# carlobaldassi/GaussDCA.jl

Hardware: AMD Instinct MI355X
Metric: end-to-end gDCA sec + achieved Cholesky TFLOP/s, N=500 M=50k q=21 (higher is better)
Workload: dtype f64

## Files before the change

### gaussdca.jl_amd/csrc/gdca_api.hip

```cpp
#include <algorithm>
#include <ctype.h>
#include <math.h>
#include <stdio.h>
#include <stdlib.h>
#include <string.h>
#include <strings.h>

#include "gdca_hamming_form.h"
#include "gdca_internal.h"
#include "gdca_launch.h"

struct gdca_buf {
    void *p;
    size_t cap;
};

class stage_pool {
    friend class host_stage;
    static const int MAX_ARRAYS = 10;
    gdca_buf buf[MAX_ARRAYS];

public:
    void release()
    {
// ... 530 lines not shown
{
    return (int32_t)sizeof(gdca_params);
}

int32_t gdca_device_count(void)
{
    int n = 0;
    if (hipGetDeviceCount(&n) != hipSuccess) return 0;
    return n;
}

gdca_status gdca_ctx_create_on_stream(int32_t device_id, void *hip_stream, gdca_ctx **out)
{
    if (!out) return GDCA_EINVAL;
    *out = nullptr;
    int ndev = 0;
    if (hipGetDeviceCount(&ndev) != hipSuccess || ndev <= 0) return GDCA_EHIP;
    if (device_id < 0 || device_id >= ndev) return GDCA_EINVAL;
    gdca_ctx *ctx = (gdca_ctx *)calloc(1, sizeof(gdca_ctx));
    if (!ctx) return GDCA_ENOMEM;
    ctx->device = device_id;
    ctx->timing = true;
    gdca_tuning_from_env(&ctx->tune);
    if (hipSetDevice(device_id) != hipSuccess) {
        free(ctx);
        return GDCA_EHIP;
    }
    ctx->stream = (hipStream_t)hip_stream;
    ctx->own_stream = false;
    {
        hipDeviceProp_t prop0;
        ctx->ncu = hipGetDeviceProperties(&prop0, device_id) == hipSuccess ? prop0.multiProcessorCount : 256;
    }
    if (hipEventCreateWithFlags(&ctx->ev_batch, hipEventDisableTiming) != hipSuccess ||
        hipEventCreateWithFlags(&ctx->ev_upload, hipEventDisableTiming) != hipSuccess) {
        gdca_ctx_destroy(ctx);
        return GDCA_EHIP;
    }
    if (hipHostMalloc((void **)&ctx->sc_host, sizeof(gdca_dev_scalars), hipHostMallocDefault) != hipSuccess) {
        ctx->sc_host = nullptr;
        gdca_ctx_destroy(ctx);
        return GDCA_ENOMEM;
    }
    if (hipHostGetDevicePointer((void **)&ctx->sc_host_dev, ctx->sc_host, 0) != hipSuccess) ctx->sc_host_dev = nullptr;
    *out = ctx;
    return GDCA_OK;
}

static gdca_status warm_stream(gdca_ctx *ctx, hipStream_t s)
{
    CHK(ensure(ctx, ctx->sc, sizeof(gdca_dev_scalars)));
    gdca_fill_async(s, ctx->sc.p, 0, sizeof(gdca_dev_scalars));
    if (hipStreamSynchronize(s) != hipSuccess) {
        (void)hipGetLastError();
        return fail(ctx, GDCA_EHIP, "the context's stream could not be started");
    }
    return GDCA_OK;
}

gdca_status gdca_ctx_create(int32_t device_id, gdca_ctx **out)
{
    gdca_status st = gdca_ctx_create_on_stream(device_id, nullptr, out);
    if (st != GDCA_OK) return st;
    gdca_ctx *ctx = *out;
    int prio_least = 0, prio_greatest = 0;
    (void)hipDeviceGetStreamPriorityRange(&prio_least, &prio_greatest);
    if (hipStreamCreateWithPriority(&ctx->stream, hipStreamNonBlocking, prio_greatest) != hipSuccess) {
        gdca_ctx_destroy(ctx);
        *out = nullptr;
        return GDCA_EHIP;
    }
    ctx->own_stream = true;
    st = warm_stream(ctx, ctx->stream);
    if (st != GDCA_OK) {
        gdca_ctx_destroy(ctx);
        *out = nullptr;
    }
    return st;
}

gdca_status gdca_ctx_create_peer(gdca_ctx *leader, gdca_ctx **out)
{
    if (!leader || !out) return GDCA_EINVAL;
    gdca_ctx *ctx = leader;
    HIPCHK(hipSetDevice(leader->device));
    if (!leader->gate) {
        gdca_gate *g = (gdca_gate *)calloc(1, sizeof(gdca_gate));
        if (!g) return GDCA_ENOMEM;
        for (int i = 0; i < 4; ++i) HIPCHK(hipEventCreateWithFlags(&g->ev[i], hipEventDisableTiming));
        g->refs = 1;
        int prio_least = 0, prio_greatest = 0;
        (void)hipDeviceGetStreamPriorityRange(&prio_least, &prio_greatest);
        if (hipStreamCreateWithPriority(&g->batch_stream, hipStreamNonBlocking, prio_greatest) != hipSuccess) g->batch_stream = nullptr;
        leader->gate = g;
    }
    const bool new_gate = leader->gate->refs == 1;
    gdca_status st = gdca_ctx_create(leader->device, out);
    if (st != GDCA_OK) return st;
    (*out)->gate = leader->gate;
    leader->gate->refs += 1;
    if (new_gate && leader->gate->batch_stream) {
        st = warm_stream(*out, leader->gate->batch_stream);
        if (st != GDCA_OK) {
            gdca_ctx_destroy(*out);
            *out = nullptr;
        }
    }
    return st;
}

gdca_status gdca_ctx_destroy(gdca_ctx *ctx)
{
    if (!ctx) return GDCA_EINVAL;
    (void)hipSetDevice(ctx->device);
    if (ctx->own_stream || ctx->stream) (void)hipStreamSynchronize(ctx->stream);
    gdca_buf *bufs[] = {&ctx->Zt, &ctx->Zp, &ctx->hist, &ctx->Zb, &ctx->hcnt, &ctx->nk, &ctx->W, &ctx->Wfix, &ctx->Pifix,
                        &ctx->Pipc, &ctx->A, &ctx->G, &ctx->H, &ctx->P, &ctx->Sg, &ctx->Dblk, &ctx->Ld,
                        &ctx->Tws, &ctx->colsum, &ctx->sc, &ctx->normws, &ctx->C2, &ctx->B0, &ctx->Rt, &ctx->Wd, &ctx->rankws, &ctx->hcand, &ctx->himg,
                        &ctx->Pij, &ctx->sc_front, &ctx->keep, &ctx->Xg, &ctx->Epart, &ctx->gpart, &ctx->gvec,
                        &ctx->PXa, &ctx->PXb, &ctx->PXpad, &ctx->PEab, &ctx->PT, &ctx->PBtab, &ctx->PBitems, &ctx->PBE,
                        &ctx->LOa, &ctx->LOb, &ctx->PBN,
                        &ctx->IPAws, &ctx->IPAcnt, &ctx->IPAZ, &ctx->IPAsel, &ctx->IPAm, &ctx->IPAg, &ctx->IPAprev, &ctx->IPAsp, &ctx->DMd, &ctx->SMst, &ctx->BMws, &ctx->BMred};
    for (gdca_buf *b : bufs)
        if (b->p) (void)hipFree(b->p);
    ctx->staging.release();
    if (ctx->gate && --ctx->gate->refs == 0) {
        for (int i = 0; i < 4; ++i) (void)hipEventDestroy(ctx->gate->ev[i]);
        if (ctx->gate->batch_stream) {
            (void)hipStreamSynchronize(ctx->gate->batch_stream);
            (void)hipStreamDestroy(ctx->gate->batch_stream);
        }
        free(ctx->gate);
    }
    for (hipEvent_t e : ctx->ev)
        if (e) (void)hipEventDestroy(e);
    if (ctx->item0_host) (void)hipHostFree(ctx->item0_host);
    if (ctx->ev_batch) (void)hipEventDestroy(ctx->ev_batch);
    if (ctx->ev_upload) (void)hipEventDestroy(ctx->ev_upload);
    if (ctx->sc_host) (void)hipHostFree(ctx->sc_host);
    if (ctx->own_stream) (void)hipStreamDestroy(ctx->stream);
    free(ctx);
    return GDCA_OK;
}

gdca_status gdca_ctx_synchronize(gdca_ctx *ctx)
{
    if (!ctx) return GDCA_EINVAL;
    HIPCHK(hipSetDevice(ctx->device));
    HIPCHK(hipStreamSynchronize(ctx->stream));
    return GDCA_OK;
}

const char *gdca_last_error(gdca_ctx *ctx)
{
    return ctx ? ctx->err : "null context";
}

gdca_status gdca_ctx_set_timing(gdca_ctx *ctx, int32_t enabled)
{
    if (!ctx) return GDCA_EINVAL;
    ctx->timing = enabled != 0;
    return GDCA_OK;
}

gdca_status gdca_ctx_set_option(gdca_ctx *ctx, const char *key, const char *value)
{
    if (!ctx) return GDCA_EINVAL;
    if (!key || !value) return fail(ctx, GDCA_EINVAL, "null option key or value");
    if (!gdca_tuning_set(&ctx->tune, key, value)) return fail(ctx, GDCA_EINVAL, "unknown option or unusable value: %s=%s", key, value);
    return GDCA_OK;
}

}

static gdca_status open_timeline(gdca_ctx *ctx, bool timed, bool stamped)
{
    gdca_pending &r = ctx->pend;
    r.timed = timed;
    r.stamped = stamped;
    r.ev_marks = r.stamp_marks = 0;
    for (int t = 0; timed && t < T_COUNT; ++t)
        if (!ctx->ev[t]) HIPCHK(hipEventCreate(&ctx->ev[t]));
    return GDCA_OK;
}

static void note_mark(gdca_pending &r, gdca_boundary t, bool stamp)
{
    (stamp ? r.stamp_marks : r.ev_marks) |= 1u << t;
    (stamp ? r.ev_marks : r.stamp_marks) &= ~(1u << t);
}

static gdca_status mark(gdca_ctx *ctx, gdca_boundary t, bool own_launch = false)
{
    gdca_pending &r = ctx->pend;
    if (!r.timed) return GDCA_OK;
    const bool stamp = r.stamped && !own_launch;
    if (stamp)
        gdca_launch_stamp(ctx->stream, (gdca_dev_scalars *)ctx->sc.p, t, T_NONE);
    else
        HIPCHK(hipEventRecord(ctx->ev[t], ctx->stream));
    note_mark(r, t, stamp);
    return GDCA_OK;
}

static gdca_status mark_members(hipStream_t s, gdca_ctx *const *mem, int K, gdca_boundary a, gdca_boundary b, bool stamps)
{
    gdca_ctx *ctx = mem[0];
    if (stamps) {
        gdca_recorder *&act = gdca_recorder::active();
        gdca_recorder *outer = act;
        if (outer) (void)outer->flush();
        gdca_recorder rec;
        rec.begin(s, K);
        for (int k = 0; k < K; ++k) {
            rec.member(k);
            gdca_launch_stamp(s, (gdca_dev_scalars *)mem[k]->sc.p, a, b);
        }
        (void)rec.end();
        act = outer;
    } else
        for (int k = 0; k < K; ++k) {
            HIPCHK(hipEventRecord(mem[k]->ev[a], s));
            HIPCHK(hipEventRecord(mem[k]->ev[b], s));
        }
    for (int k = 0; k < K; ++k) {
        note_mark(mem[k]->pend, a, stamps);
        note_mark(mem[k]->pend, b, stamps);
    }
    return GDCA_OK;
}

static void sweep_events(gdca_ctx *ctx, hipEvent_t *begin, hipEvent_t *end)
{
    const bool timed = ctx->pend.timed;
    *begin = timed ? ctx->ev[T_SWEEP_BEGIN] : nullptr;
    *end = timed ? ctx->ev[T_SWEEP_END] : nullptr;
    note_mark(ctx->pend, T_SWEEP_BEGIN, false);
    note_mark(ctx->pend, T_SWEEP_END, false);
}

static double elapsed(const gdca_ctx *ctx, gdca_boundary a, gdca_boundary b, bool *failed)
{
    const gdca_pending &r = ctx->pend;
    const unsigned both = 1u << a | 1u << b;
    if (!r.timed) return 0.0;
    if ((r.stamp_marks & both) == both) return (double)(long long)(ctx->sc_host->stamp[b] - ctx->sc_host->stamp[a]) * 1e-5;
    if ((r.ev_marks & both) != both) return 0.0;
    float ms = 0.f;
    if (hipEventElapsedTime(&ms, ctx->ev[a], ctx->ev[b]) != hipSuccess) *failed = true;
    return ms;
}

static hipError_t gate_wait(const gdca_gate *g, hipStream_t s)
{
    return g->armed ? hipStreamWaitEvent(s, g->ev[g->last], 0) : hipSuccess;
}

static hipError_t gate_pass(gdca_gate *g, hipStream_t s)
{
    const hipError_t e = hipEventRecord(g->ev[g->next], s);
    if (e != hipSuccess) return e;
    g->last = g->next;
    g->next = (g->next + 1) & 3;
    g->armed = 1;
    return hipSuccess;
}

static gdca_status member_error(gdca_ctx *lead, gdca_ctx *m, int k, gdca_status st)
{
    if (k > 0 && m != lead && m->err[0]) {
        char msg[sizeof(lead->err)];
        snprintf(msg, sizeof(msg), "member %d: %.400s", k, m->err);
        memcpy(lead->err, msg, sizeof(msg));
    }
    return st;
}

static gdca_status upload_done(gdca_ctx *ctx)
{
    HIPCHK(hipEventRecord(ctx->ev_upload, ctx->stream));
    HIPCHK(hipEventSynchronize(ctx->ev_upload));
    return GDCA_OK;
}

static double inverse_flops_model(double n)
{
    return (n * n * n / 3.0 + n * n / 2.0 + n / 6.0) + (2.0 * n * n * n / 3.0 + n * n / 2.0 + 5.0 * n / 6.0);
}

static int round_up(int x, int m)
{
    return (x + m - 1) / m * m;
}

static gdca_status weights_stage(gdca_ctx *ctx, const int8_t *Zd, int N, int M, int q, double theta_in, int fixed_thresh,
                                 bool want_theta_only)
{
    hipStream_t s = ctx->stream;
    gdca_dev_scalars *sc = (gdca_dev_scalars *)ctx->sc.p;
    CHK(ensure(ctx, ctx->hist, gdca_column_hist_bytes(N, M)));
    if (fixed_thresh >= 0) {
        gdca_launch_set_thresh(s, sc, fixed_thresh);
    } else {
        if (theta_in < 0.0) gdca_launch_column_hist(s, Zd, (uint32_t *)ctx->hist.p, N, M);
        gdca_launch_theta_finalize(s, (const uint32_t *)ctx->hist.p, N, M, theta_in, sc);
    }
    CHK(check_launch(ctx, "theta"));
    CHK(mark(ctx, T_THETA));
    if (want_theta_only) return GDCA_OK;

    const int Mt = (M + GDCA_HTILE - 1) / GDCA_HTILE;
    CHK(ensure(ctx, ctx->Zb, gdca_bitplane_bytes(N, M)));
    CHK(ensure(ctx, ctx->hcnt, (size_t)Mt * GDCA_HTILE * sizeof(int32_t)));
    if (!ctx->tune.force_fallback && ctx->tune.hamming_mode != 0) CHK(ensure(ctx, ctx->hcand, gdca_hamming_cand_cap(M) * 8));
    const bool fp4 = !ctx->tune.force_fallback && (ctx->tune.hamming_mode == 2 || (ctx->tune.hamming_mode < 0 && gdca_hamming_consensus_gate(N, M)));
    if (fp4) CHK(ensure(ctx, ctx->himg, gdca_fp4_image_bytes(N, M)));
    CHK(ensure(ctx, ctx->nk, (size_t)M * sizeof(int32_t)));
    CHK(ensure(ctx, ctx->W, (size_t)M * sizeof(double)));
    CHK(ensure(ctx, ctx->Wfix, (size_t)M * sizeof(unsigned long long)));
    gdca_fill_async(s, ctx->hcnt.p, 0, (size_t)Mt * GDCA_HTILE * sizeof(int32_t));
    gdca_launch_bitplane_pack(s, Zd, (uint32_t *)ctx->Zb.p, N, M, q, sc);
    if (ctx->tune.force_fallback) {
        gdca_launch_hamming_fallback(s, Zd, (int32_t *)ctx->hcnt.p, N, M, sc);
    } else {
        if (fp4) {
            if (!(fixed_thresh < 0 && theta_in < 0.0)) gdca_launch_column_hist(s, Zd, (uint32_t *)ctx->hist.p, N, M);
            gdca_launch_hamming_fp4_image(s, Zd, (const uint32_t *)ctx->hist.p, ctx->himg.p, N, M);
        }
        gdca_launch_hamming(s, (const uint32_t *)ctx->Zb.p, Zd, (int32_t *)ctx->hcnt.p, N, M, sc, ctx->tune.hamming_mode, ctx->hcand.p, fp4 ? ctx->himg.p : nullptr, ctx->tune.ham_cut);
    }
    gdca_launch_weights(s, (const int32_t *)ctx->hcnt.p, M, gdca_fix_shift(M), (int32_t *)ctx->nk.p,
                        (double *)ctx->W.p, (unsigned long long *)ctx->Wfix.p);
    gdca_launch_meff(s, (const double *)ctx->W.p, M, sc);
    return check_launch(ctx, "weights");
}

static gdca_status tally_stage(gdca_ctx *ctx, const int8_t *Zd, int N, int M, int q, const double *Meff_dev, double pc,
                               int mode, double *Pi_true_out, double *out, size_t ld, bool want_norm1 = false)
{
    hipStream_t s = ctx->stream;
    const int sdim = q - 1, n = N * sdim;
    const int shift = gdca_fix_shift(M);
    const int TJ = gdca_tally_tj(q, ctx->tune.tally_tj);
    const bool skip = gdca_tally_skip(q, TJ, ctx->tune.tally_skip, M);
    const size_t keep_list = (size_t)N * M * sizeof(uint32_t);
    if (skip) CHK(ensure(ctx, ctx->keep, keep_list + (size_t)N * sizeof(int) + N));
    CHK(ensure(ctx, ctx->Zt, (size_t)N * M + 3));
    CHK(ensure(ctx, ctx->Zp, (size_t)round_up(N, 64) * M + 64));
    CHK(ensure(ctx, ctx->Pifix, (size_t)N * 32 * sizeof(unsigned long long)));
    CHK(ensure(ctx, ctx->Pipc, (size_t)n * sizeof(double)));
    uint32_t *keep = skip ? (uint32_t *)ctx->keep.p : nullptr;
    int *keep_n = skip ? (int *)((char *)ctx->keep.p + keep_list) : nullptr;
    uint8_t *sigma = skip ? (uint8_t *)(keep_n + N) : nullptr;
    gdca_launch_relayout(s, Zd, (int8_t *)ctx->Zt.p, (int8_t *)ctx->Zp.p, N, M, TJ);
    gdca_launch_pi_keep(s, (const int8_t *)ctx->Zt.p, (const unsigned long long *)ctx->Wfix.p, (unsigned long long *)ctx->Pifix.p, keep, keep_n,
                        sigma, N, M, q, (gdca_dev_scalars *)ctx->sc.p);
    gdca_launch_pi_finalize(s, (const unsigned long long *)ctx->Pifix.p, N, q, shift, Meff_dev, pc, Pi_true_out,
                            (double *)ctx->Pipc.p, want_norm1 ? &((gdca_dev_scalars *)ctx->sc.p)->pi_max : nullptr);
    if (want_norm1) CHK(mark(ctx, T_TALLY_BEGIN));
    gdca_launch_pair_tally(s, (const int8_t *)ctx->Zp.p, (const int8_t *)ctx->Zt.p,
                           (const unsigned long long *)ctx->Wfix.p, N, M, q, shift, Meff_dev, pc,
                           (const double *)ctx->Pipc.p, mode, out, ld, TJ, keep, keep_n, sigma,
                           (const unsigned long long *)ctx->Pifix.p);
    if (want_norm1) CHK(mark(ctx, T_TALLY_END));
    if (want_norm1 && !gdca_norm1_settled(N, q, pc, ctx->tune.refine, ctx->tune.refine_cond))
        gdca_launch_cov_norm1(s, out, ld, N, q, pc, ctx->tune.refine_cond, (gdca_dev_scalars *)ctx->sc.p, ctx->tune.refine == 1);
    return check_launch(ctx, "tally");
}

static gdca_status inverse_job(gdca_ctx *ctx, int n, int n_pad, gdca_inverse_job *job)
{
    const size_t pbytes = (size_t)n_pad * GDCA_TILE * sizeof(double);
    const int nblk = n_pad / GDCA_TILE;
    const size_t sg = (size_t)4 * GDCA_TILE * 4 * GDCA_TILE * sizeof(double);
    const size_t fbytes = gdca_inverse_flag_bytes(n_pad);
    CHK(ensure(ctx, ctx->G, (size_t)8 * pbytes));
    CHK(ensure(ctx, ctx->H, (size_t)8 * pbytes));
    CHK(ensure(ctx, ctx->P, (size_t)GDCA_TILE * GDCA_TILE * sizeof(double)));
    const size_t piv_off = (4 * sg + fbytes + (size_t)3 * (nblk + 2) * sizeof(int) + 15) & ~(size_t)15;
    CHK(ensure(ctx, ctx->Sg, piv_off + (size_t)n_pad * sizeof(double)));
    if (ctx->item0_cap < 3 * (nblk + 2)) {
        if (ctx->item0_host) HIPCHK(hipHostFree(ctx->item0_host));
        ctx->item0_host = nullptr;
        ctx->item0_cap = 0;
        HIPCHK(hipHostMalloc((void **)&ctx->item0_host, (size_t)3 * (nblk + 2) * sizeof(int), hipHostMallocDefault));
        ctx->item0_cap = 3 * (nblk + 2);
    }
    gdca_inverse_ws &ws = job->ws;
    for (int w = 0; w < 8; ++w) {
        ws.G[w] = (double *)((char *)ctx->G.p + (size_t)w * pbytes);
        ws.H[w] = (double *)((char *)ctx->H.p + (size_t)w * pbytes);
    }
    ws.P = (double *)ctx->P.p;
    ws.Sg[0] = (double *)ctx->Sg.p;
    ws.Sg[1] = (double *)((char *)ctx->Sg.p + sg);
    ws.Pg[0] = (double *)((char *)ctx->Sg.p + 2 * sg);
    ws.Pg[1] = (double *)((char *)ctx->Sg.p + 3 * sg);
    ws.flags = (unsigned *)((char *)ctx->Sg.p + 4 * sg);
    ws.flags_bytes = fbytes;
    ws.item0_dev = (int *)((char *)ctx->Sg.p + 4 * sg + fbytes);
    ws.item0_host = ctx->item0_host;
    ws.piv = ctx->piv = (double *)((char *)ctx->Sg.p + piv_off);
    ctx->ld.count = 0;
    ctx->ld.chol = false;
    {
        void *dp = nullptr;
        ws.item0_host_dev = hipHostGetDevicePointer(&dp, ctx->item0_host, 0) == hipSuccess ? (const int *)dp : nullptr;
    }
    ws.update_cus = ctx->ncu;
    job->A = (double *)ctx->A.p;
    job->n_pad = n_pad;
    job->n_real = n;
    job->sc = (gdca_dev_scalars *)ctx->sc.p;
    job->tune = &ctx->tune;
    job->doomed = (ctx->tune.sweep_debug & 32) != 0 && ctx->pend.at.attempt == 0;
    return GDCA_OK;
}

static gdca_status poison_inverse_ws(gdca_ctx *ctx, hipStream_t s)
{
    HIPCHK(hipMemsetAsync(ctx->G.p, 0xFF, ctx->G.cap, s));
    HIPCHK(hipMemsetAsync(ctx->H.p, 0xFF, ctx->H.cap, s));
    HIPCHK(hipMemsetAsync(ctx->P.p, 0xFF, ctx->P.cap, s));
    HIPCHK(hipMemsetAsync(ctx->Sg.p, 0xFF, (size_t)4 * 4 * GDCA_TILE * 4 * GDCA_TILE * sizeof(double), s));
    return GDCA_OK;
}

static gdca_status inverse_stage(gdca_ctx *ctx, int n, int n_pad, double *upd_flops)
{
    gdca_inverse_job job;
    CHK(inverse_job(ctx, n, n_pad, &job));
    hipEvent_t sweep_begin, sweep_end;
    sweep_events(ctx, &sweep_begin, &sweep_end);
    if (ctx->tune.sweep_debug & 16) CHK(poison_inverse_ws(ctx, ctx->stream));
    if (ctx->tune.sweep_debug & 8) {
        double fl = 0.0;
        gdca_launch_spd_inverse_merged(ctx->stream, &job, 1, sweep_begin, sweep_end, &fl);
        if (upd_flops) *upd_flops = fl;
        return check_launch(ctx, "spd_inverse_merged");
    }
    gdca_launch_spd_inverse(ctx->stream, job, sweep_begin, sweep_end, upd_flops);
    return check_launch(ctx, "spd_inverse");
}

static gdca_status logdet_stage(gdca_ctx *ctx, int n)
{
    gdca_launch_logdet(ctx->stream, ctx->piv, n, (gdca_dev_scalars *)ctx->sc.p);
    return check_launch(ctx, "logdet");
}

static void note_logdet(gdca_ctx *ctx, int k = 0)
{
    const gdca_dev_scalars &h = *ctx->sc_host;
    ctx->ld.val[k] = h.info == 0 && !h.bad_symbol ? h.logdet : (double)NAN;
    ctx->ld.src[k] = ctx->ld.chol ? 1 : 0;
    ctx->ld.count = k + 1;
}

static gdca_status g_room(gdca_ctx *ctx, int n)
{
    const int nb = gdca_energy_gblocks(n);
    CHK(ensure(ctx, ctx->gpart, (size_t)nb * nb * 64 * sizeof(double)));
    return ensure(ctx, ctx->gvec, ((size_t)n + 1) * sizeof(double));
}

static void g_launch(gdca_ctx *ctx, const gdca_model &m)
{
    const int n = m.N * (m.q - 1);
    double *g = (double *)ctx->gvec.p;
    gdca_launch_energy_g(ctx->stream, m.A, m.ld, m.sign, n, m.Pi, (double *)ctx->gpart.p, g, g + n);
}

static gdca_status pack_and_g(gdca_ctx *ctx, const gdca_model &m, const int8_t *X_dev, int K, size_t stride = 0)
{
    CHK(ensure(ctx, ctx->Xg, (size_t)gdca_energy_blocks(m.N) * K * sizeof(uint32_t)));
    CHK(g_room(ctx, m.N * (m.q - 1)));
    gdca_launch_energy_pack(ctx->stream, X_dev, stride ? stride : (size_t)m.N, m.N, K, m.q, (uint32_t *)ctx->Xg.p, (gdca_dev_scalars *)ctx->sc.p);
    g_launch(ctx, m);
    return GDCA_OK;
}

static gdca_status energy_stage(gdca_ctx *ctx, const gdca_model &m, const int8_t *X_dev, int K, double *E_dev, size_t stride = 0)
{
    const int sdim = m.q - 1, n = m.N * sdim;
    const int Kc = gdca_energy_chunk(m.N, K, ctx->tune.energy_chunk);
    CHK(ensure(ctx, ctx->Epart, (size_t)gdca_energy_blocks(m.N) * Kc * sizeof(double)));
    CHK(pack_and_g(ctx, m, X_dev, K, stride));
    const double *g = (const double *)ctx->gvec.p;
    for (int k0 = 0; k0 < K; k0 += Kc)
        HIPCHK(gdca_launch_energy_rows(ctx->stream, m.A, m.ld, m.sign, g, g + n, (const uint32_t *)ctx->Xg.p, m.N, sdim, K, k0,
                                       std::min(Kc, K - k0), (double *)ctx->Epart.p, E_dev, ctx->ncu));
    return check_launch(ctx, "energies");
}

static gdca_status pair_pack(gdca_ctx *ctx, int N, int q, int split, const int8_t *XA, size_t strideA, int KA, const int8_t *XB, size_t strideB,
                             int KB, int what)
{
    hipStream_t s = ctx->stream;
    gdca_dev_scalars *sc = (gdca_dev_scalars *)ctx->sc.p;
    CHK(ensure(ctx, ctx->PXa, (size_t)gdca_energy_blocks(split) * KA * sizeof(uint32_t)));
    CHK(ensure(ctx, ctx->PXb, (size_t)gdca_energy_blocks(N - split) * KB * sizeof(uint32_t)));
    gdca_launch_energy_pack(s, XA, strideA, split, KA, q, (uint32_t *)ctx->PXa.p, sc);
    gdca_launch_energy_pack(s, XB, strideB, N - split, KB, q, (uint32_t *)ctx->PXb.p, sc);
    if (what == GDCA_PAIR_ENERGY) {
        CHK(ensure(ctx, ctx->PXpad, (size_t)N * ((size_t)KA + (size_t)KB)));
        gdca_launch_pair_pad(s, XA, strideA, XB, strideB, N, split, KA, KB, q, (int8_t *)ctx->PXpad.p);
    }
    return GDCA_OK;
}

static gdca_status pair_stage(gdca_ctx *ctx, const gdca_model &m, int split, const int8_t *XA, size_t strideA, int KA, const int8_t *XB,
                              size_t strideB, int KB, int what, double *E_dev, const pair_blocks *blk = nullptr, bool packed = false,
                              const gdca_logodds_terms *lo = nullptr)
{
    hipStream_t s = ctx->stream;
    const int N = m.N, q = m.q, sdim = q - 1, n = N * sdim, nB = (N - split) * sdim;
    if (!packed) CHK(pair_pack(ctx, N, q, split, XA, strideA, KA, XB, strideB, KB, what));
    const double *EAB = nullptr, *c0 = nullptr;
    if (what == GDCA_PAIR_ENERGY) {
        CHK(ensure(ctx, ctx->PEab, ((size_t)KA + (size_t)KB) * sizeof(double)));
        CHK(energy_stage(ctx, m, (const int8_t *)ctx->PXpad.p, KA + KB, (double *)ctx->PEab.p));
        EAB = (const double *)ctx->PEab.p;
        c0 = (const double *)ctx->gvec.p + n;
    }
    const int Ac = blk ? blk->Ac : gdca_pair_chunk(nB, KA, ctx->tune.pair_chunk);
    CHK(ensure(ctx, ctx->PT, (size_t)Ac * nB * sizeof(double)));
    for (int a0 = 0, c = 0; a0 < KA; a0 += Ac, ++c) {
        if (blk)
            HIPCHK(gdca_launch_pair_chunk_blocked(s, m.A, m.ld, m.sign, (const uint32_t *)ctx->PXa.p, (const uint32_t *)ctx->PXb.p, N, split, sdim,
                                                  KA, KB, a0, std::min(Ac, KA - a0), (double *)ctx->PT.p, EAB, c0, E_dev,
                                                  blk->items + 4 * blk->first[c], blk->first[c + 1] - blk->first[c], blk->eoff, blk->offA,
                                                  blk->offB, ctx->ncu, lo));
        else
            HIPCHK(gdca_launch_pair_chunk(s, m.A, m.ld, m.sign, (const uint32_t *)ctx->PXa.p, (const uint32_t *)ctx->PXb.p, N, split, sdim, KA, KB,
                                          a0, std::min(Ac, KA - a0), (double *)ctx->PT.p, EAB, c0, E_dev, ctx->ncu, lo));
    }
    return check_launch(ctx, blk ? "blocked pair energies" : "pair energies");
}

static gdca_status assign_stage(gdca_ctx *ctx, const double *E_dev, const pair_blocks &blk, int32_t *match_dev, double *gap_dev)
{
    HIPCHK(gdca_launch_assign_blocks(ctx->stream, E_dev, blk.eoff, blk.offA, blk.offB, blk.S, blk.kmax, match_dev, gap_dev));
    return check_launch(ctx, "assignment");
}

static gdca_status mutation_stage(gdca_ctx *ctx, const gdca_model &m, const int8_t *X_dev, int K, int what, double *D_dev)
{
    CHK(pack_and_g(ctx, m, X_dev, K));
    HIPCHK(gdca_launch_mutation_scan(ctx->stream, m.A, m.ld, m.sign, (const double *)ctx->gvec.p, (const uint32_t *)ctx->Xg.p, m.N, m.q - 1, K,
                                     what, D_dev, ctx->ncu));
    return check_launch(ctx, "mutation scan");
}

static gdca_status double_stage(gdca_ctx *ctx, const gdca_model &m, const int8_t *X_dev, int K, double *Emin_dev, int32_t *code_dev,
                                double *epi_dev, const int32_t *muts_dev, int L, double *out_dev)
{
    CHK(ensure(ctx, ctx->DMd, (size_t)m.q * (size_t)m.N * (size_t)K * sizeof(double)));
    CHK(mutation_stage(ctx, m, X_dev, K, GDCA_MUT_DELTA, (double *)ctx->DMd.p));
    if (muts_dev) {
        gdca_launch_double_mutants(ctx->stream, m.A, m.ld, m.sign, (const uint32_t *)ctx->Xg.p, (const double *)ctx->DMd.p, muts_dev, L, m.N,
                                   m.q - 1, K, out_dev, (gdca_dev_scalars *)ctx->sc.p);
        return check_launch(ctx, "double mutants");
    }
    HIPCHK(gdca_launch_double_mutant_scan(ctx->stream, m.A, m.ld, m.sign, (const uint32_t *)ctx->Xg.p, (const double *)ctx->DMd.p, m.N, m.q - 1,
                                          K, Emin_dev, code_dev, epi_dev, ctx->tune.epi_generic != 0));
    return check_launch(ctx, "double-mutant scan");
}

static bool walk_placement(const gdca_ctx *ctx, int N, int q, bool *in_lds)
{
    const bool fits = gdca_walk_table_fits(N, q);
    *in_lds = ctx->tune.walk_table == 2 ? false : fits;
    return fits || ctx->tune.walk_table != 1;
}

static gdca_status walk_stage(gdca_ctx *ctx, const gdca_model &m, const int8_t *X_dev, int K, const walk_request &w)
{
    bool in_lds = false;
    if (!walk_placement(ctx, m.N, m.q, &in_lds)) return fail(ctx, GDCA_EINVAL, "WALK_TABLE = lds: the table does not fit into LDS");
    double *V = w.V;
    if (!V) {
        CHK(ensure(ctx, ctx->DMd, (size_t)m.q * (size_t)m.N * (size_t)K * sizeof(double)));
        V = (double *)ctx->DMd.p;
    }
    CHK(mutation_stage(ctx, m, X_dev, K, GDCA_MUT_POTENTIAL, V));
    HIPCHK(gdca_launch_greedy_walk(ctx->stream, m.A, m.ld, m.sign, (const uint32_t *)ctx->Xg.p, m.N, m.q - 1, K, w.mask, w.flags, w.min_gain,
                                   w.max_steps, V, in_lds, w.V != nullptr, w.Xout, w.steps, w.dE_sum, w.path, w.dE_path));
    return check_launch(ctx, "greedy walk");
}

static gdca_status sample_stage(gdca_ctx *ctx, const gdca_model &m, const int8_t *X_dev, int K, const sample_request &r)
{
    bool in_lds = false;
    if (!walk_placement(ctx, m.N, m.q, &in_lds)) return fail(ctx, GDCA_EINVAL, "WALK_TABLE = lds: the table does not fit into LDS");
    double *V = r.V;
    if (!V) {
        CHK(ensure(ctx, ctx->DMd, (size_t)m.q * (size_t)m.N * (size_t)K * sizeof(double)));
        V = (double *)ctx->DMd.p;
    }
    CHK(ensure(ctx, ctx->SMst, gdca_sample_state_bytes(m.N, K)));
    CHK(mutation_stage(ctx, m, X_dev, K, GDCA_MUT_POTENTIAL, V));
    const int n_steps = r.plan.burn + r.plan.n_samples * r.plan.stride;
    const int chunk = ctx->tune.sample_chunk > 0 ? ctx->tune.sample_chunk : GDCA_SAMPLE_CHUNK_RULE;
    for (int t0 = 0; t0 < n_steps;) {
        const int t1 = n_steps - t0 > chunk ? t0 + chunk : n_steps;
        HIPCHK(gdca_launch_sample(ctx->stream, m.A, m.ld, m.sign, (const uint32_t *)ctx->Xg.p, m.N, m.q - 1, K, r.plan, t0, t1, V, in_lds,
                                  ctx->SMst.p));
        t0 = t1;
    }
    return check_launch(ctx, "Metropolis chains");
}

static gdca_status score_stage(gdca_ctx *ctx, int N, int sdim, int n_pad, const score_target &t)
{
    hipStream_t s = ctx->stream;
    const gdca_model m{(const double *)ctx->A.p, (size_t)n_pad, -1.0, (const double *)ctx->Pipc.p + (size_t)ctx->pend.site0 * sdim, N, sdim + 1};
    if (t.logodds) return GDCA_OK;
    switch (t.kind) {
    case score_target::ENERGY:
    case score_target::LOGLIK: return energy_stage(ctx, m, t.X, t.K, t.out, t.strideX);
    case score_target::PAIR: return pair_stage(ctx, m, t.split, t.XA, t.strideA, t.KA, t.XB, t.strideB, t.KB, t.what, t.out);
    case score_target::PARTNER:
        CHK(pair_stage(ctx, m, t.split, t.XA, t.strideA, t.KA, t.XB, t.strideB, t.KB, t.what, t.out, &t.blocks, t.packed));
        return assign_stage(ctx, t.out, t.blocks, t.match, t.gap);
    case score_target::MUTATION: return mutation_stage(ctx, m, t.X, t.K, t.what, t.out);
    case score_target::DOUBLE_SCAN: return double_stage(ctx, m, t.X, t.K, t.out, t.dcode, t.depi, nullptr, 0, nullptr);
    case score_target::DOUBLE_LIST: return double_stage(ctx, m, t.X, t.K, nullptr, nullptr, nullptr, t.muts, t.L, t.out);
    case score_target::WALK: return walk_stage(ctx, m, t.X, t.K, t.walk);
    case score_target::SAMPLE: return sample_stage(ctx, m, t.X, t.K, t.sample);
    case score_target::CONTACT: break;
    }
    double *S_dev = t.out;
    if (t.score == GDCA_SCORE_DI) {
        CHK(ensure(ctx, ctx->Tws, gdca_di_ws_bytes(N, sdim)));
        gdca_launch_di(s, (const double *)ctx->A.p, (size_t)n_pad, (const double *)ctx->Ld.p, N, sdim, S_dev,
                       (double *)ctx->Tws.p, (gdca_dev_scalars *)ctx->sc.p);
// ... 2942 lines not shown
```

### gaussdca.jl_amd/csrc/gdca_internal.h

```cpp
#pragma once

#include <hip/hip_runtime.h>
#include <stdint.h>

#include <vector>

#include "gdca.h"
#include "gdca_inverse_outcome.h"

#define GDCA_TILE 128
#define GDCA_HTILE 128
#define GDCA_MAXQ 31

enum gdca_boundary {
    T_NONE = -1,
    T_BEGIN, T_THETA, T_WEIGHTS,
    T_TALLY_BEGIN, T_TALLY_END,
    T_COV,
    T_INV_BEGIN, T_SWEEP_BEGIN, T_SWEEP_END, T_INV_END,
    T_SCORE_BEGIN, T_FN_BEGIN, T_FN_END, T_END,
    T_COUNT
};

struct gdca_dev_scalars {
    double theta;
    double Meff;
    unsigned long long pair_sum;
    int thresh;
    int info;
    int bad_symbol;
    int di_noconv;
    int ham_mode;
    int ham_cand;
    unsigned long long ham_ncand;
    unsigned long long sweep_cycles, sweep_ticks;
    double inv_norm1;
    double ns_resid;
    double mat_norm1;
    double pi_max;
    unsigned long long stamp[T_COUNT];
    int ham_cand2;
    int ham_cut;
    unsigned ham_alive[64];
    double logdet;
};

struct gdca_tuning {
    int group;
    int ramp;
    int ragged;
    int rem_tail;
    int panel_halves;
    int slab;
    int ring;
    int mcus;
    int mcu_solo;
    int sweep_debug;
    long sweep_timeout_ms;
    int sweep_retries;
    int tally_tj;
    int tally_skip;
    int hamming_mode;
    int ham_cut;
    int force_fallback;
    int merge;
    int merge_blocks;
    int merge_mcus;
    int merge_group;
    int merge_tiles;
    int phased_fronts;
    int phased_grids;
    int phased_streams;
    int refine;
    double refine_cond;
    int cholesky;
    int energy_chunk;
    int pair_chunk;
    int epi_generic;
    int walk_table;
    int sample_chunk;
    char sweep_trace[256];
};
void gdca_tuning_from_env(gdca_tuning *t);
bool gdca_tuning_set(gdca_tuning *t, const char *key, const char *value);

void gdca_launch_relayout(hipStream_t s, const int8_t *Z, int8_t *Zt, int8_t *Zc, int N, int M, int TJ);
size_t gdca_column_hist_bytes(int N, int M);
void gdca_launch_column_hist(hipStream_t s, const int8_t *Z, uint32_t *cnt, int N, int M);
void gdca_launch_theta_finalize(hipStream_t s, const uint32_t *cnt, int N, int M, double theta_in,
                                gdca_dev_scalars *sc);
void gdca_launch_set_thresh(hipStream_t s, gdca_dev_scalars *sc, int thresh);

size_t gdca_bitplane_bytes(int N, int M);
void gdca_launch_bitplane_pack(hipStream_t s, const int8_t *Z, uint32_t *Zb, int N, int M, int q,
                               gdca_dev_scalars *sc);
size_t gdca_hamming_cand_cap(int M);
size_t gdca_fp4_image_bytes(int N, int M);
void gdca_launch_hamming_fp4_image(hipStream_t s, const int8_t *Z, const uint32_t *hist, void *img, int N, int M);
void gdca_launch_hamming_fp4_probe(hipStream_t s, const void *img, int N, int M, int nprobe, gdca_dev_scalars *sc);
void gdca_launch_hamming_fp4(hipStream_t s, const void *img, int N, int M, gdca_dev_scalars *sc, void *cand_list, unsigned cap);
void gdca_launch_hamming(hipStream_t s, const uint32_t *Zb, const int8_t *Z, int32_t *cnt, int N, int M, gdca_dev_scalars *sc, int force,
                         void *cand_list, void *fp4_img, int cut);
void gdca_launch_hamming_fallback(hipStream_t s, const int8_t *Z, int32_t *cnt, int N, int M, const gdca_dev_scalars *sc);
void gdca_launch_weights(hipStream_t s, const int32_t *cnt, int M, int fix_shift, int32_t *n_out, double *W,
                         unsigned long long *Wfix);
void gdca_launch_meff(hipStream_t s, const double *W, int M, gdca_dev_scalars *sc);
void gdca_launch_fix_weights(hipStream_t s, const double *W, int M, int fix_shift, unsigned long long *Wfix,
                             gdca_dev_scalars *sc);
int gdca_fix_shift(int M);

void gdca_launch_pi_keep(hipStream_t s, const int8_t *Zt, const unsigned long long *Wfix, unsigned long long *Pifix, uint32_t *keep,
                         int *keep_n, uint8_t *sigma, int N, int M, int q, gdca_dev_scalars *sc);
void gdca_launch_pi_finalize(hipStream_t s, const unsigned long long *Pifix, int N, int q, int fix_shift,
                             const double *Meff_dev, double pc, double *Pi_true, double *Pi_pc, double *pi_max = nullptr);
void gdca_launch_cov_norm1(hipStream_t s, const double *C, size_t ld, int N, int q, double pc, double cond_limit, gdca_dev_scalars *sc,
                           int always);
int gdca_tally_tj(int q, int tj_wanted);
bool gdca_tally_skip(int q, int TJ, int skip_wanted, int M);
void gdca_launch_pair_tally(hipStream_t s, const int8_t *Zc, const int8_t *Zt, const unsigned long long *Wfix,
                            int N, int M, int q, int fix_shift, const double *Meff_dev, double pc,
                            const double *Pi_pc, int mode, double *out, size_t ld, int TJ, const uint32_t *keep = nullptr,
                            const int *keep_n = nullptr, const uint8_t *sigma = nullptr, const unsigned long long *Pifix = nullptr);
void gdca_launch_cov_from_pij(hipStream_t s, const double *Pij, const double *Pi_pc, int N, int q, double pc, double *out, size_t ld,
                              size_t ldp = 0);

void gdca_launch_add_pseudocount(hipStream_t s, const double *Pi_true, const double *Pij_true, int N, int q,
                                 double pc, double *Pi, double *Pij);
void gdca_launch_covariance(hipStream_t s, const double *Pi, const double *Pij, int n, double *C);
void gdca_launch_pad_identity(hipStream_t s, double *A, int n, int n_pad);
void gdca_launch_copy_in(hipStream_t s, const double *src, int n, double *dst, int n_pad);
void gdca_launch_copy_in_neg(hipStream_t s, const double *src, int n, double *dst, int n_pad);
void gdca_launch_copy_out_neg_sym(hipStream_t s, const double *A, int n_pad, double *dst, int n);
void gdca_launch_publish_scalars(hipStream_t s, const gdca_dev_scalars *sc, gdca_dev_scalars *host_mapped);
void gdca_launch_save_diag_blocks(hipStream_t s, const double *C, size_t ld, int N, int sdim, double *D);

struct gdca_inverse_ws {
    double *G[8];
    double *H[8];
    double *P;
    double *piv;
    double *Sg[2];
    double *Pg[2];
    unsigned *flags;
    size_t flags_bytes;
    int *item0_host;
    const int *item0_host_dev;
    int *item0_dev;
    int update_cus;
};
struct gdca_inverse_job {
    double *A;
    int n_pad, n_real;
    gdca_inverse_ws ws;
    gdca_dev_scalars *sc;
    const gdca_tuning *tune;
    bool doomed;
};
size_t gdca_inverse_flag_bytes(int n_pad);
void gdca_launch_spd_inverse(hipStream_t s, const gdca_inverse_job &job, hipEvent_t sweep_begin, hipEvent_t sweep_end, double *upd_flops);
int gdca_inverse_max_merge(void);
void gdca_launch_spd_inverse_merged(hipStream_t s, const gdca_inverse_job *jobs, int K, hipEvent_t sweep_begin, hipEvent_t sweep_end,
                                    double *upd_flops);
size_t gdca_ranking_ws_bytes(long long len);
void gdca_launch_ranking(hipStream_t s, const double *S_dev, int N, int sep, long long len, void *ws, int32_t **ii, int32_t **jj, double **sc);
__device__ __forceinline__ uint64_t gdca_rank_key(double x)
{
    const uint64_t u = (uint64_t)__double_as_longlong(x);
    uint64_t asc = (u >> 63) ? ~u : (u | 0x8000000000000000ull);
    if (x != x) asc = ~0ull;
    return ~asc;
}
size_t gdca_sort_hist_words(size_t n);
void gdca_launch_sort_pairs(hipStream_t s, uint64_t *const key[2], uint32_t *const val[2], uint32_t *hist, size_t n);
void gdca_launch_probe_mfma_f64(hipStream_t s, double *out, int iters, int blocks);
void gdca_launch_cholesky_inverse(hipStream_t s, double *C2, double *U, double *Tm, double *Wd, double *Aout, int n_pad, int n_real,
                                  gdca_dev_scalars *sc, double *piv);
void gdca_launch_inverse_norm1(hipStream_t s, const double *A, int n_pad, int n, double *colsum_ws, double *out);
void gdca_launch_matrix_norm1(hipStream_t s, const double *C, size_t ld, int n, double *colsum_ws, double *out);
void gdca_launch_newton_schulz(hipStream_t s, double *A, const double *C2, double *B0, double *Rt, int n_pad, double *resid);

void gdca_launch_logdet(hipStream_t s, const double *piv, int n_real, gdca_dev_scalars *sc);
void gdca_launch_loglik(hipStream_t s, double *L, int K, double c);

void gdca_launch_fn(hipStream_t s, const double *A, size_t ld, int N, int sdim, double *S, int ncu = 0);
void gdca_launch_diag_chol(hipStream_t s, const double *D, int N, int sdim, double *Ld);
size_t gdca_di_ws_bytes(int N, int sdim);
void gdca_launch_di(hipStream_t s, const double *A, size_t ld, const double *Ld, int N, int sdim, double *S,
                    double *Tws, gdca_dev_scalars *sc);
void gdca_launch_apc(hipStream_t s, double *S, int N, double *rowsum_ws);

struct gdca_model {
    const double *A;
    size_t ld;
    double sign;
    const double *Pi;
    int N, q;
};

int gdca_energy_blocks(int Ns);
int gdca_energy_gblocks(int n);
int gdca_energy_chunk(int N, int K, int wanted);
void gdca_launch_energy_pack(hipStream_t s, const int8_t *X, size_t stride, int Ns, int K, int q, uint32_t *Xg, gdca_dev_scalars *sc);
void gdca_launch_energy_g(hipStream_t s, const double *A, size_t ld, double sign, int n, const double *Pi, double *part, double *g,
                          double *c0);
hipError_t gdca_launch_energy_rows(hipStream_t s, const double *A, size_t ld, double sign, const double *g, const double *c0,
                                   const uint32_t *Xg, int N, int sdim, int K, int k0, int Kc, double *part, double *E, int ncu);

int gdca_pair_chunk(int nB, int KA, int wanted);
void gdca_launch_pair_pad(hipStream_t s, const int8_t *XA, size_t strideA, const int8_t *XB, size_t strideB, int N, int split, int KA, int KB,
                          int q, int8_t *Xp);
struct gdca_logodds_terms {
    const double *EmA, *EmB;
    double I;
};
hipError_t gdca_launch_pair_chunk(hipStream_t s, const double *A, size_t ld, double sign, const uint32_t *XAg, const uint32_t *XBg, int N,
                                  int split, int sdim, int KA, int KB, int a0, int Ac, double *T, const double *EAB, const double *c0, double *E,
                                  int ncu, const gdca_logodds_terms *lo = nullptr);
void gdca_pair_block_items(const int32_t *offA, const int32_t *offB, int S, int Ac, std::vector<int32_t> &items, std::vector<long long> &first);
hipError_t gdca_launch_pair_chunk_blocked(hipStream_t s, const double *A, size_t ld, double sign, const uint32_t *XAg, const uint32_t *XBg, int N,
                                          int split, int sdim, int KA, int KB, int a0, int Ac, double *T, const double *EAB, const double *c0,
                                          double *E, const int32_t *items, long long nitems, const long long *eoff, const int32_t *offA,
                                          const int32_t *offB, int ncu, const gdca_logodds_terms *lo = nullptr);
void gdca_launch_negate(hipStream_t s, const double *src, double *dst, size_t len);

hipError_t gdca_launch_assign_blocks(hipStream_t s, const double *E, const long long *eoff, const int32_t *offA, const int32_t *offB, int S,
                                     int kmax, int32_t *match, double *gap);

struct gdca_ipa_counts {
    double cost;
    int n_changed;
    int ncand;
    int n_sel;
    int pad_;
};
size_t gdca_ipa_select_ws_bytes(int KA);
void gdca_launch_ipa_select(hipStream_t s, const int32_t *match, const double *gap, int KA, int n_take, void *ws, int32_t *sel, gdca_ipa_counts *out);
void gdca_launch_ipa_concat(hipStream_t s, const int8_t *XA, int KA, const int8_t *XB, int KB, int N, int split, const int32_t *selA,
                            const int32_t *selB, const int32_t *viaB, int n_sel, int8_t *Z, size_t col0, gdca_dev_scalars *sc);
void gdca_launch_ipa_round(hipStream_t s, const double *E, const long long *eoff, const int32_t *offA, const int32_t *offB, const int32_t *spA,
                           const int32_t *match, const int32_t *prev, int KA, gdca_ipa_counts *out);
void gdca_launch_ipa_publish(hipStream_t s, const int32_t *match, const double *gap, int KA, int32_t *prev, int32_t *match_out, double *gap_out,
                             int32_t *match_row, double *gap_row);

hipError_t gdca_launch_mutation_scan(hipStream_t s, const double *A, size_t ld, double sign, const double *g, const uint32_t *Xg, int N, int sdim,
                               int K, int what, double *D, int ncu);

#define GDCA_EPI_MAX_GROUPS (1LL << 24)
hipError_t gdca_launch_double_mutant_scan(hipStream_t s, const double *A, size_t ld, double sign, const uint32_t *Xg, const double *D, int N,
                                          int sdim, int K, double *Emin, int32_t *code, double *epi, bool generic);
void gdca_launch_double_mutants(hipStream_t s, const double *A, size_t ld, double sign, const uint32_t *Xg, const double *D,
                                const int32_t *muts, long long L, int N, int sdim, int K, double *out, gdca_dev_scalars *sc);

#define GDCA_WALK_LDS_LIMIT (160 * 1024)
size_t gdca_walk_lds_bytes(int N, int q, bool table_in_lds);
bool gdca_walk_table_fits(int N, int q);
hipError_t gdca_launch_greedy_walk(hipStream_t s, const double *A, size_t ld, double sign, const uint32_t *Xg, int N, int sdim, int K,
                                   const int8_t *mask, int flags, double min_gain, int max_steps, double *V, bool table_in_lds, bool write_table,
                                   int8_t *Xout, int32_t *steps, double *dE_sum, int32_t *path, double *dE_path);

#define GDCA_SAMPLE_CHUNK_RULE 65536
struct gdca_sample_plan {
    const int8_t *mask;
    int flags;
    double beta;
    unsigned long long seed, stream0;
    int burn, stride, n_samples;
    int8_t *Xs;
    double *dE_s;
    int32_t *accepted;
    double *thr;
    int32_t *moves;
};
size_t gdca_sample_lds_bytes(int N, int q, bool table_in_lds);
size_t gdca_sample_state_bytes(int N, int K);
hipError_t gdca_launch_sample(hipStream_t s, const double *A, size_t ld, double sign, const uint32_t *Xg, int N, int sdim, int K,
                              const gdca_sample_plan &plan, int t0, int t1, double *V, bool table_in_lds, void *state);

void gdca_launch_bm_from_gaussian(hipStream_t s, const double *mJ, const double *g, int N, int sdim, double *W);
void gdca_launch_bm_update(hipStream_t s, double *W, const double *Pij_d, const double *Pij_m, int N, int sdim, double eta, double lambda);
size_t gdca_bm_readout_bytes(int n);
void gdca_launch_bm_readout(hipStream_t s, const double *Pi_d, const double *Pij_d, const double *Pi_m, const double *Pij_m, int N, int sdim,
                            double *part, double *out, bool zero3);
void gdca_launch_bm_accept(hipStream_t s, const int32_t *accepted, int K, long long n_steps, double *out);
void gdca_launch_bm_last_sample(hipStream_t s, const int8_t *Xs, int N, int K, int n_samples, int8_t *X);
void gdca_launch_bm_fill(hipStream_t s, double *v, size_t count, double value);
```

### gaussdca.jl_amd/csrc/k_hamming.hip

```cpp
#include <algorithm>
#include <cstdlib>

#include "gdca_hamming_cut.h"
#include "gdca_hamming_form.h"
#include "gdca_internal.h"
#include "gdca_launch.h"

#define NPLANES 5
#define WCHUNK 8

size_t gdca_bitplane_bytes(int N, int M)
{
    const size_t Mt = (M + GDCA_HTILE - 1) / GDCA_HTILE, NW = (N + 31) / 32;
    return Mt * NPLANES * NW * GDCA_HTILE * sizeof(uint32_t);
}

struct k_bitplane_pack_args {
    const int8_t *Z;
    uint32_t *Zb;
    int N;
    int M;
    int NW;
    int q;
    gdca_dev_scalars *sc;
};
static inline k_bitplane_pack_args k_bitplane_pack_mk(const int8_t *Z, uint32_t *Zb, int N, int M, int NW, int q, gdca_dev_scalars *sc)
{
    return k_bitplane_pack_args{Z, Zb, N, M, NW, q, sc};
}
template <int CAP>
__global__ __launch_bounds__(128) void k_bitplane_pack(const BatchArgs<k_bitplane_pack_args, CAP> B_)
{
    GDCA_MEMBER(B_);
    const int8_t *__restrict__ Z = a_.Z;
    uint32_t *__restrict__ Zb = a_.Zb;
    int N = a_.N;
    int M = a_.M;
    int NW = a_.NW;
    int q = a_.q;
    gdca_dev_scalars *sc = a_.sc;
    uint32_t bad = 0;
    const uint32_t over = (0x7fu - (uint32_t)q) * 0x01010101u;
    const int tile = blockIdx.x, w = blockIdx.y, kl = threadIdx.x;
    const int k = tile * GDCA_HTILE + kl;
    uint32_t pl[NPLANES];
#pragma unroll
    for (int p = 0; p < NPLANES; ++p) pl[p] = 0;
    if (k < M) {
        const int8_t *src = Z + (size_t)k * N + (size_t)w * 32;
        const int nb = min(32, N - w * 32);
        if (nb == 32 && (N & 3) == 0) {
            const uint32_t *s4 = reinterpret_cast<const uint32_t *>(src);
            uint32_t d[8];
#pragma unroll
            for (int j = 0; j < 8; ++j) d[j] = s4[j];
#pragma unroll
            for (int j = 0; j < 8; ++j) {
                bad |= (d[j] - 0x01010101u) & ~d[j] & 0x80808080u;
                bad |= (((d[j] & 0x7f7f7f7fu) + over) | d[j]) & 0x80808080u;
            }
#pragma unroll
            for (int j = 0; j < 8; ++j)
#pragma unroll
                for (int p = 0; p < NPLANES; ++p) {
                    const uint32_t t = (d[j] >> p) & 0x01010101u;
                    pl[p] |= (((t * 0x01020408u) >> 24) & 0xFu) << (4 * j);
                }
        } else {
            for (int b = 0; b < nb; ++b) {
                const uint32_t raw = (uint32_t)(uint8_t)src[b];
                bad |= (raw - 1u) >= (uint32_t)q;
                const uint32_t z = raw & 31u;
#pragma unroll
                for (int p = 0; p < NPLANES; ++p) pl[p] |= ((z >> p) & 1u) << b;
            }
        }
    }
#pragma unroll
    for (int p = 0; p < NPLANES; ++p)
        Zb[(((size_t)tile * NPLANES + p) * NW + w) * GDCA_HTILE + kl] = pl[p];
    if (bad) atomicOr(&sc->bad_symbol, GDCA_BAD_ALIGNMENT);
}

void gdca_launch_bitplane_pack(hipStream_t s, const int8_t *Z, uint32_t *Zb, int N, int M, int q, gdca_dev_scalars *sc)
{
    const int Mt = (M + GDCA_HTILE - 1) / GDCA_HTILE, NW = (N + 31) / 32;
    (gdca_launch<k_bitplane_pack_args, k_bitplane_pack<1>, k_bitplane_pack<GDCA_MAXB>>(dim3(Mt, NW), dim3(128), 0, s, k_bitplane_pack_mk(Z, Zb, N, M, NW, q, sc)));
}

__device__ __forceinline__ void tri_decode(int t, int Mt, int &I, int &J)
{
    const double b = 2.0 * Mt + 1.0;
    int i = (int)((b - sqrt(b * b - 8.0 * (double)t)) * 0.5);
    if (i < 0) i = 0;
    if (i > Mt - 1) i = Mt - 1;
    auto start = [Mt](int r) { return (long long)r * Mt - (long long)r * (r - 1) / 2; };
    while (i > 0 && start(i) > t) --i;
    while (i < Mt - 1 && start(i + 1) <= t) ++i;
    I = i;
    J = i + (int)(t - start(i));
}

#define HAM_BOUND_PLANES 3
#define HAM_CAND_CAP 1024

__shared__ int hm_any[3];
__shared__ unsigned hm_tile_n, hm_tile_base;
__shared__ uint32_t hm_list[4][HAM_LIST_WAVE];
__shared__ int hm_wave_n[4];
__shared__ unsigned hm_alive[HAM_ALIVE_SLOTS];
#define HAM_ENT_DIST 0x3ffffu
#define HAM_NO_PAIR 0x40000000u
static_assert(sizeof(((gdca_dev_scalars *)nullptr)->ham_alive) == HAM_ALIVE_SLOTS * sizeof(unsigned), "one slot per word the probe counts");
__device__ __forceinline__ bool wg_any(bool pred, int &k)
{
    const int s = k % 3, n = (k + 1) % 3;
    ++k;
    if (threadIdx.x == 0) hm_any[n] = 0;
    if (__any(pred) && (threadIdx.x & 63) == 0) atomicOr(&hm_any[s], 1);
    __syncthreads();
    return hm_any[s] != 0;
}


size_t gdca_hamming_cand_cap(int M)
{
    const long long Mt = (M + GDCA_HTILE - 1) / GDCA_HTILE;
    return (size_t)std::min<long long>(Mt * (Mt + 1) / 2 * HAM_CAND_PER_TILE + 4096, 1ll << 30);
}

struct k_hamming_refine_args {
    const int8_t *Z;
    const int2 *list;
    unsigned cap;
    int N;
    int32_t *cnt;
    const gdca_dev_scalars *sc;
};
static inline k_hamming_refine_args k_hamming_refine_mk(const int8_t *Z, const int2 *list, unsigned cap, int N, int32_t *cnt, const gdca_dev_scalars *sc)
{
    return k_hamming_refine_args{Z, list, cap, N, cnt, sc};
}
template <int CAP>
__global__ __launch_bounds__(256) void k_hamming_refine(const BatchArgs<k_hamming_refine_args, CAP> B_)
{
    GDCA_MEMBER(B_);
    const int8_t *__restrict__ Z = a_.Z;
    const int2 *__restrict__ list = a_.list;
    unsigned cap = a_.cap;
    int N = a_.N;
    int32_t *__restrict__ cnt = a_.cnt;
    const gdca_dev_scalars *__restrict__ sc = a_.sc;
    if (sc->ham_mode == 0) return;
    if (sc->ham_ncand > (unsigned long long)cap) return;
    const unsigned total = (unsigned)sc->ham_ncand;
    const int thresh = sc->thresh;
    const int tid = threadIdx.x, sub = tid & 15, grp = (tid & 63) >> 4;
    const unsigned wave = blockIdx.x * 4u + (unsigned)(tid >> 6), nwave = gridDim.x * 4u;
    for (unsigned eb = wave * 4u; eb < total; eb += nwave * 4u) {
        const unsigned e = eb + (unsigned)grp;
        uint32_t d = 0;
        int k = 0, l = 0;
        if (e < total) {
            const int2 pr = list[e];
            k = pr.x;
            l = pr.y;
            const int8_t *zk = Z + (size_t)k * N, *zl = Z + (size_t)l * N;
            if ((N & 3) == 0 && (reinterpret_cast<uintptr_t>(Z) & 3) == 0) {
                const uint32_t *a = reinterpret_cast<const uint32_t *>(zk), *b = reinterpret_cast<const uint32_t *>(zl);
                const int nw = N >> 2;
                for (int w0 = 0; w0 < nw; w0 += 256) {
                    uint32_t xa[16], xb[16];
#pragma unroll
                    for (int u = 0; u < 16; ++u) {
                        const int w = w0 + 16 * u + sub;
                        xa[u] = w < nw ? a[w] : 0u;
                        xb[u] = w < nw ? b[w] : 0u;
                    }
#pragma unroll
                    for (int u = 0; u < 16; ++u) {
                        uint32_t x = xa[u] ^ xb[u];
                        x |= x >> 4;
                        x |= x >> 2;
                        x |= x >> 1;
                        d += __builtin_popcount(x & 0x01010101u);
                    }
                }
            } else {
                for (int i = sub; i < N; i += 16) d += zk[i] != zl[i];
            }
        }
        d += __shfl_xor(d, 1);
        d += __shfl_xor(d, 2);
        d += __shfl_xor(d, 4);
        d += __shfl_xor(d, 8);
        if (e < total && sub == 0 && (int)d < thresh) {
            atomicAdd(&cnt[k], 1);
            atomicAdd(&cnt[l], 1);
        }
    }
}

struct k_hamming_args {
    const uint32_t *Zb;
    int32_t *cnt;
    int NW;
    int M;
    int Mt;
    gdca_dev_scalars *sc;
    int2 *cand_list;
    unsigned cand_cap;
};
static inline k_hamming_args k_hamming_mk(const uint32_t *Zb, int32_t *cnt, int NW, int M, int Mt, gdca_dev_scalars *sc, int2 *cand_list, unsigned cand_cap)
{
    return k_hamming_args{Zb, cnt, NW, M, Mt, sc, cand_list, cand_cap};
}
template <int CAP, int NP, bool PROBE>
__global__ __launch_bounds__(256, (NP < NPLANES && !PROBE) ? 4 : 3) void k_hamming(const BatchArgs<k_hamming_args, CAP> B_)
{
    GDCA_MEMBER(B_);
    const uint32_t *__restrict__ Zb = a_.Zb;
    int32_t *__restrict__ cnt = a_.cnt;
    int NW = a_.NW;
    int M = a_.M;
    int Mt = a_.Mt;
    gdca_dev_scalars *__restrict__ sc = a_.sc;
    int2 *__restrict__ cand_list = a_.cand_list;
    unsigned cand_cap = a_.cand_cap;
    const int thresh = sc->thresh;
    if (thresh <= 0) return;
    if constexpr (!PROBE) {
        const bool mine = NP == NPLANES ? (sc->ham_mode == 0 || sc->ham_ncand > cand_cap) : sc->ham_mode == 1;
        if (!mine) return;
    }

    __shared__ __attribute__((aligned(16))) uint32_t As[NP][WCHUNK][GDCA_HTILE];
    __shared__ __attribute__((aligned(16))) uint32_t Bs[NP][WCHUNK][GDCA_HTILE];
    __shared__ int rc[GDCA_HTILE], cc[GDCA_HTILE];

    int I, J;
    tri_decode(PROBE ? (int)(((long long)blockIdx.x * ((long long)Mt * (Mt + 1) / 2)) / gridDim.x) : (int)blockIdx.x, Mt, I, J);
    const int tid = threadIdx.x, tx = tid & 15, ty = tid >> 4;
    if (tid < GDCA_HTILE) {
        rc[tid] = 0;
        cc[tid] = 0;
    }
    if (tid == 0) {
        hm_any[0] = 0;
        hm_any[1] = 0;
        hm_tile_n = 0u;
    }
    int any_calls = 0;

    uint32_t acc[8][8];
#pragma unroll
    for (int r = 0; r < 8; ++r)
#pragma unroll
        for (int c = 0; c < 8; ++c) acc[r][c] = 0;
    if constexpr (NP < NPLANES) {
        if (I == J || (J + 1) * GDCA_HTILE > M) {
#pragma unroll
            for (int r = 0; r < 8; ++r)
#pragma unroll
                for (int c = 0; c < 8; ++c) {
                    const int lc = (c < 4) ? (tx * 4 + c) : (64 + tx * 4 + (c - 4));
                    const int gr = I * GDCA_HTILE + ty * 8 + r, gc = J * GDCA_HTILE + lc;
                    acc[r][c] = (gr < M && gc < M && (I == J ? (PROBE ? gr != gc : gr < gc) : true)) ? 0u : HAM_NO_PAIR;
                }
        }
    }
    bool all_beyond = false;

    const uint32_t *Ag = Zb + (size_t)I * NPLANES * NW * GDCA_HTILE;
    const uint32_t *Bg = Zb + (size_t)J * NPLANES * NW * GDCA_HTILE;

    constexpr bool CUTTING = NP < NPLANES && !PROBE;
    int cut = NW;
    if constexpr (CUTTING) {
        const int c = sc->ham_cut;
        if (c > 0 && c < NW && NW < HAM_CUT_MAX_NW) cut = c;
    }
    bool sparse = false;
    if constexpr (PROBE)
        if (tid < HAM_ALIVE_SLOTS) hm_alive[tid] = 0u;

    auto stage = [&](int w0) {
#pragma unroll
        for (int p = 0; p < NP; ++p) {
            const int wl = tid >> 5;
            uint4 va = make_uint4(0, 0, 0, 0), vb = make_uint4(0, 0, 0, 0);
            if (w0 + wl < NW) {
                const size_t off = ((size_t)p * NW + w0 + wl) * GDCA_HTILE + (size_t)(tid & 31) * 4;
                va = *reinterpret_cast<const uint4 *>(Ag + off);
                vb = *reinterpret_cast<const uint4 *>(Bg + off);
            }
            *reinterpret_cast<uint4 *>(&As[p][wl][(tid & 31) * 4]) = va;
            *reinterpret_cast<uint4 *>(&Bs[p][wl][(tid & 31) * 4]) = vb;
        }
    };

    int w0 = 0;
    for (; w0 < NW; w0 += WCHUNK) {
        __syncthreads();
        stage(w0);
        __syncthreads();
        const int wn = min(WCHUNK, NW - w0);
        int w = 0;
        bool again;
        do {
        again = false;
        for (const int wend = CUTTING ? min(wn, cut - w0) : wn; w < wend; ++w) {
            uint32_t a[NP][8], b[NP][8];
#pragma unroll
            for (int p = 0; p < NP; ++p) {
                const uint4 a0 = *reinterpret_cast<const uint4 *>(&As[p][w][ty * 8]);
                const uint4 a1 = *reinterpret_cast<const uint4 *>(&As[p][w][ty * 8 + 4]);
                const uint4 b0 = *reinterpret_cast<const uint4 *>(&Bs[p][w][tx * 4]);
                const uint4 b1 = *reinterpret_cast<const uint4 *>(&Bs[p][w][64 + tx * 4]);
                a[p][0] = a0.x; a[p][1] = a0.y; a[p][2] = a0.z; a[p][3] = a0.w;
                a[p][4] = a1.x; a[p][5] = a1.y; a[p][6] = a1.z; a[p][7] = a1.w;
                b[p][0] = b0.x; b[p][1] = b0.y; b[p][2] = b0.z; b[p][3] = b0.w;
                b[p][4] = b1.x; b[p][5] = b1.y; b[p][6] = b1.z; b[p][7] = b1.w;
            }
#pragma unroll
            for (int r = 0; r < 8; ++r)
#pragma unroll
                for (int c = 0; c < 8; ++c) {
                    uint32_t x = a[0][r] ^ b[0][c];
#pragma unroll
                    for (int p = 1; p < NP; ++p)
                        x = __builtin_amdgcn_bitop3_b32(a[p][r], b[p][c], x, 0xBE);
                    acc[r][c] += __builtin_popcount(x);
                }
            if constexpr (PROBE) {
                if (w0 + w < HAM_ALIVE_SLOTS) {
                    int alive = 0;
#pragma unroll
                    for (int r = 0; r < 8; ++r)
#pragma unroll
                        for (int c = 0; c < 8; ++c) alive += __builtin_popcountll(__ballot((int)acc[r][c] < thresh));
                    if ((tid & 63) == 0 && alive) atomicAdd(&hm_alive[w0 + w], (unsigned)alive);
                }
            }
        }
        if constexpr (CUTTING) {
            if (w0 + w == cut && cut < NW) {
                const uint32_t rc0 = ((uint32_t)(ty * 8) << 25) | ((uint32_t)(tx * 4) << 18);
                uint32_t *const mylist = hm_list[tid >> 6];
                int wcount = 0;
#pragma unroll
                for (int r = 0; r < 8; ++r)
#pragma unroll
                    for (int c = 0; c < 8; ++c) {
                        const bool lv = (int)acc[r][c] < thresh;
                        const unsigned long long m = __ballot(lv);
                        if (m != 0ull) {
                            if (lv) {
                                const int pos = wcount + (int)__builtin_amdgcn_mbcnt_hi((unsigned)(m >> 32), __builtin_amdgcn_mbcnt_lo((unsigned)m, 0u));
                                const uint32_t rc = ((uint32_t)r << 25) | ((uint32_t)((c < 4) ? c : 64 + (c - 4)) << 18);
                                if (pos < HAM_LIST_WAVE) mylist[pos] = acc[r][c] + (rc0 + rc);
                            }
                            wcount += __builtin_popcountll(m);
                        }
                    }
                if ((tid & 63) == 0) hm_wave_n[tid >> 6] = wcount;
                __syncthreads();
                const int n0 = hm_wave_n[0], n1 = hm_wave_n[1], n2 = hm_wave_n[2], n3 = hm_wave_n[3];
                if (max(max(n0, n1), max(n2, n3)) > HAM_LIST_WAVE) {
                    cut = NW;
                    again = w < wn;
                } else if ((n0 | n1 | n2 | n3) == 0) {
                    all_beyond = true;
                } else {
                    sparse = true;
                }
            }
        }
        } while (again);
        if (CUTTING && (sparse || all_beyond)) break;
        if (w0 + WCHUNK < NW) {
            uint32_t mn = acc[0][0];
#pragma unroll
            for (int r = 0; r < 8; ++r)
#pragma unroll
                for (int c = 0; c < 8; ++c) mn = min(mn, acc[r][c]);
            if (!wg_any((int)mn < thresh, any_calls)) {
                all_beyond = true;
                break;
            }
        }
    }

    const bool diag = (I == J);
    if constexpr (PROBE) {
        int cand = 0;
#pragma unroll
        for (int r = 0; r < 8; ++r)
#pragma unroll
            for (int c = 0; c < 8; ++c) {
                const int lc = (c < 4) ? (tx * 4 + c) : (64 + tx * 4 + (c - 4));
                const int gr = I * GDCA_HTILE + ty * 8 + r, gc = J * GDCA_HTILE + lc;
                cand += (gr < M) && (gc < M) && (gr != gc) && ((int)acc[r][c] < thresh);
            }
        if (cand) atomicAdd(&rc[0], cand);
        __syncthreads();
        if (tid == 0 && rc[0]) atomicAdd(&sc->ham_cand, rc[0]);
        if (tid < HAM_ALIVE_SLOTS && hm_alive[tid]) atomicAdd(&sc->ham_alive[tid], hm_alive[tid]);
        return;
    }
    if (all_beyond) return;
    if constexpr (CUTTING) {
        if (sparse) {
            const int lane = tid & 63, nmine = hm_wave_n[tid >> 6];
            uint32_t *const mylist = hm_list[tid >> 6];
            for (int ws = cut; ws < NW; ws = w0 + WCHUNK) {
                if (ws >= w0 + WCHUNK) {
                    w0 += WCHUNK;
                    __syncthreads();
                    stage(w0);
                    __syncthreads();
                }
                const int wn = min(WCHUNK, NW - w0);
                bool left = false;
                for (int e = lane; e < nmine; e += 64) {
                    const uint32_t ent = mylist[e];
                    uint32_t d = ent & HAM_ENT_DIST;
                    if ((int)d < thresh) {
                        const int row = (int)(ent >> 25), col = (int)((ent >> 18) & 127u);
                        for (int w = ws - w0; w < wn; ++w) {
                            uint32_t x = As[0][w][row] ^ Bs[0][w][col];
#pragma unroll
                            for (int p = 1; p < NP; ++p) x = __builtin_amdgcn_bitop3_b32(As[p][w][row], Bs[p][w][col], x, 0xBE);
                            d += __builtin_popcount(x);
                        }
                        mylist[e] = (ent & ~HAM_ENT_DIST) | d;
                        left |= (int)d < thresh;
                    }
                }
                if (w0 + WCHUNK < NW && !wg_any(left, any_calls)) return;
            }
            unsigned mine = 0u;
            for (int e = lane; e < nmine; e += 64) mine += (int)(mylist[e] & HAM_ENT_DIST) < thresh;
            if (!wg_any(mine != 0u, any_calls)) return;
            const unsigned off = mine ? atomicAdd(&hm_tile_n, mine) : 0u;
            __syncthreads();
            if (tid == 0) {
                const unsigned long long base = atomicAdd(&sc->ham_ncand, (unsigned long long)hm_tile_n);
                hm_tile_base = base > (unsigned long long)cand_cap ? cand_cap : (unsigned)base;
            }
            __syncthreads();
            unsigned slot = hm_tile_base + off;
            for (int e = lane; e < nmine; e += 64) {
                const uint32_t ent = mylist[e];
                if ((int)(ent & HAM_ENT_DIST) < thresh) {
                    if (slot < cand_cap) cand_list[slot] = make_int2(I * GDCA_HTILE + (int)(ent >> 25), J * GDCA_HTILE + (int)((ent >> 18) & 127u));
                    ++slot;
                }
            }
            return;
        }
    }
    if constexpr (NP < NPLANES) {
        uint32_t mn = acc[0][0];
#pragma unroll
        for (int r = 0; r < 8; ++r)
#pragma unroll
            for (int c = 0; c < 8; ++c) mn = min(mn, acc[r][c]);
        unsigned long long cand = 0ull;
        if ((int)mn < thresh) {
#pragma unroll
            for (int r = 0; r < 8; ++r)
#pragma unroll
                for (int c = 0; c < 8; ++c) {
                    const int lc = (c < 4) ? (tx * 4 + c) : (64 + tx * 4 + (c - 4));
                    const int gr = I * GDCA_HTILE + ty * 8 + r, gc = J * GDCA_HTILE + lc;
                    if ((int)acc[r][c] < thresh && gr < M && gc < M && (diag ? gr < gc : true)) cand |= 1ull << (8 * r + c);
                }
        }
        if (!wg_any(cand != 0ull, any_calls)) return;
        const unsigned mine = (unsigned)__builtin_popcountll(cand);
        const unsigned off = mine ? atomicAdd(&hm_tile_n, mine) : 0u;
        __syncthreads();
        if (tid == 0) {
            const unsigned long long base = atomicAdd(&sc->ham_ncand, (unsigned long long)hm_tile_n);
            hm_tile_base = base > (unsigned long long)cand_cap ? cand_cap : (unsigned)base;
        }
        __syncthreads();
        unsigned slot = hm_tile_base + off;
        while (cand) {
            const int e = __builtin_ctzll(cand), r = e >> 3, c = e & 7;
            const int lc = (c < 4) ? (tx * 4 + c) : (64 + tx * 4 + (c - 4));
            if (slot < cand_cap) cand_list[slot] = make_int2(I * GDCA_HTILE + ty * 8 + r, J * GDCA_HTILE + lc);
            ++slot;
            cand &= cand - 1;
        }
        return;
    }

    if constexpr (NP == NPLANES) {
        int rowc[8], colc[8];
#pragma unroll
        for (int r = 0; r < 8; ++r) rowc[r] = 0;
#pragma unroll
        for (int c = 0; c < 8; ++c) colc[c] = 0;
#pragma unroll
        for (int r = 0; r < 8; ++r) {
            const int gr = I * GDCA_HTILE + ty * 8 + r;
#pragma unroll
            for (int c = 0; c < 8; ++c) {
                const int lc = (c < 4) ? (tx * 4 + c) : (64 + tx * 4 + (c - 4));
                const int gc = J * GDCA_HTILE + lc;
                const bool ok = (gr < M) && (gc < M) && (gr != gc) && ((int)acc[r][c] < thresh);
                rowc[r] += ok ? 1 : 0;
                colc[c] += ok ? 1 : 0;
            }
        }
#pragma unroll
        for (int r = 0; r < 8; ++r)
            if (rowc[r]) atomicAdd(&rc[ty * 8 + r], rowc[r]);
        if (!diag) {
#pragma unroll
            for (int c = 0; c < 8; ++c) {
                const int lc = (c < 4) ? (tx * 4 + c) : (64 + tx * 4 + (c - 4));
                if (colc[c]) atomicAdd(&cc[lc], colc[c]);
            }
        }
    }
    __syncthreads();
    if (tid < GDCA_HTILE) {
        const int v = rc[tid];
        if (v) atomicAdd(&cnt[I * GDCA_HTILE + tid], v);
    } else if (!diag) {
        const int v = cc[tid - GDCA_HTILE];
        if (v) atomicAdd(&cnt[J * GDCA_HTILE + tid - GDCA_HTILE], v);
    }
}

struct k_hamming_decide_args {
    gdca_dev_scalars *sc;
    long long sampled_pairs;
    int force;
    int consensus;
    int N, M;
    int cut;
};
static inline k_hamming_decide_args k_hamming_decide_mk(gdca_dev_scalars *sc, long long sampled_pairs, int force, int consensus, int N, int M, int cut)
{
    return k_hamming_decide_args{sc, sampled_pairs, force, consensus, N, M, cut};
}
template <int CAP>
__global__ void k_hamming_decide(const BatchArgs<k_hamming_decide_args, CAP> B_)
{
    GDCA_MEMBER(B_);
    gdca_dev_scalars *sc = a_.sc;
    long long sampled_pairs = a_.sampled_pairs;
    int force = a_.force;
    if (threadIdx.x == 0 && blockIdx.x == 0) {
        const double pairs = (double)sampled_pairs;
        const int NW = (a_.N + 31) / 32;
        const int cut = a_.cut > 0 ? a_.cut : (force < 0 ? gdca_hamming_pick_cut(sc->ham_alive, pairs, NW) : NW);
        sc->ham_cut = cut;
        sc->ham_mode = force >= 0 ? force : gdca_hamming_pick_form((double)sc->ham_cand, a_.consensus ? (double)sc->ham_cand2 : -1.0, pairs, a_.N, a_.M, cut);
        sc->ham_ncand = 0u;
    }
}

void gdca_launch_hamming(hipStream_t s, const uint32_t *Zb, const int8_t *Z, int32_t *cnt, int N, int M, gdca_dev_scalars *sc, int force,
                         void *cand_list, void *fp4_img, int cut)
{
    const int Mt = (M + GDCA_HTILE - 1) / GDCA_HTILE, NW = (N + 31) / 32;
    const long long ntile = (long long)Mt * (Mt + 1) / 2;
    int2 *list = (int2 *)cand_list;
    const unsigned cap = (unsigned)gdca_hamming_cand_cap(M);
    const int nprobe = (int)std::min<long long>(ntile, 192);
    if (force == 2 && !fp4_img) force = 1;
    if (force < 0 && NW <= 2) force = 0;
    if (force < 0 && ntile >= 64) {
        (gdca_launch<k_hamming_args, k_hamming<1, HAM_BOUND_PLANES, true>, k_hamming<GDCA_MAXB, HAM_BOUND_PLANES, true>>(dim3((unsigned)nprobe), dim3(256), 0, s, k_hamming_mk(Zb, cnt, NW, M, Mt, sc, list, cap)));
        if (fp4_img) gdca_launch_hamming_fp4_probe(s, fp4_img, N, M, nprobe, sc);
        (gdca_launch<k_hamming_decide_args, k_hamming_decide<1>, k_hamming_decide<GDCA_MAXB>>(dim3(1), dim3(1), 0, s, k_hamming_decide_mk(sc, (long long)nprobe * GDCA_HTILE * GDCA_HTILE, -1, fp4_img ? 1 : 0, N, M, cut)));
    } else {
        (gdca_launch<k_hamming_decide_args, k_hamming_decide<1>, k_hamming_decide<GDCA_MAXB>>(dim3(1), dim3(1), 0, s, k_hamming_decide_mk(sc, 1ll, force < 0 ? 0 : force, 0, N, M, cut)));
    }
    const bool decided = !(force < 0 && ntile >= 64);
    const int form = decided ? (force < 0 ? 0 : force) : -1;
    if (fp4_img && (form == 2 || form < 0)) gdca_launch_hamming_fp4(s, fp4_img, N, M, sc, list, cap);
    if (form == 1 || form < 0)
        (gdca_launch<k_hamming_args, k_hamming<1, HAM_BOUND_PLANES, false>, k_hamming<GDCA_MAXB, HAM_BOUND_PLANES, false>>(dim3((unsigned)ntile), dim3(256), 0, s, k_hamming_mk(Zb, cnt, NW, M, Mt, sc, list, cap)));
    if (form != 0)
        (gdca_launch<k_hamming_refine_args, k_hamming_refine<1>, k_hamming_refine<GDCA_MAXB>>(dim3(2048), dim3(256), 0, s, k_hamming_refine_mk(Z, (const int2 *)list, cap, N, cnt, (const gdca_dev_scalars *)sc)));
    (gdca_launch<k_hamming_args, k_hamming<1, NPLANES, false>, k_hamming<GDCA_MAXB, NPLANES, false>>(dim3((unsigned)ntile), dim3(256), 0, s, k_hamming_mk(Zb, cnt, NW, M, Mt, sc, list, cap)));
}

struct k_hamming_bytes_args {
    const int8_t *Z;
    int32_t *cnt;
    int N;
    int M;
    const gdca_dev_scalars *sc;
};
static inline k_hamming_bytes_args k_hamming_bytes_mk(const int8_t *Z, int32_t *cnt, int N, int M, const gdca_dev_scalars *sc)
{
    return k_hamming_bytes_args{Z, cnt, N, M, sc};
}
template <int CAP>
__global__ __launch_bounds__(256) void k_hamming_bytes(const BatchArgs<k_hamming_bytes_args, CAP> B_)
{
    GDCA_MEMBER(B_);
    const int8_t *__restrict__ Z = a_.Z;
    int32_t *__restrict__ cnt = a_.cnt;
    int N = a_.N;
    int M = a_.M;
    const gdca_dev_scalars *sc = a_.sc;
    extern __shared__ int8_t zk[];
    __shared__ int red[256];
    const int k = blockIdx.x, tid = threadIdx.x, thresh = sc->thresh;
    for (int i = tid; i < N; i += 256) zk[i] = Z[(size_t)k * N + i];
    __syncthreads();
    int mine = 0;
    for (int l = tid; l < M; l += 256) {
        if (l == k) continue;
        const int8_t *zl = Z + (size_t)l * N;
        int d = 0;
        for (int i = 0; i < N; ++i) d += (zl[i] != zk[i]);
        mine += (d < thresh);
    }
    red[tid] = mine;
    __syncthreads();
    for (int w = 128; w > 0; w >>= 1) {
        if (tid < w) red[tid] += red[tid + w];
        __syncthreads();
    }
    if (tid == 0) cnt[k] = red[0];
}

void gdca_launch_hamming_fallback(hipStream_t s, const int8_t *Z, int32_t *cnt, int N, int M, const gdca_dev_scalars *sc)
{
    (gdca_launch<k_hamming_bytes_args, k_hamming_bytes<1>, k_hamming_bytes<GDCA_MAXB>>(dim3((unsigned)M), dim3(256), (size_t)N, s, k_hamming_bytes_mk(Z, cnt, N, M, sc)));
}

int gdca_fix_shift(int M)
{
    int lg = 0;
    while ((1ll << lg) < (long long)M) ++lg;
    const int sh = 63 - lg;
    return sh < 58 ? sh : 58;
}

struct k_weights_args {
    const int32_t *cnt;
    int M;
    int fix_shift;
    int32_t *n_out;
    double *W;
    unsigned long long *Wfix;
};
static inline k_weights_args k_weights_mk(const int32_t *cnt, int M, int fix_shift, int32_t *n_out, double *W, unsigned long long *Wfix)
{
    return k_weights_args{cnt, M, fix_shift, n_out, W, Wfix};
}
template <int CAP>
__global__ __launch_bounds__(256) void k_weights(const BatchArgs<k_weights_args, CAP> B_)
{
    GDCA_MEMBER(B_);
    const int32_t *__restrict__ cnt = a_.cnt;
    int M = a_.M;
    int fix_shift = a_.fix_shift;
    int32_t *__restrict__ n_out = a_.n_out;
    double *__restrict__ W = a_.W;
    unsigned long long *__restrict__ Wfix = a_.Wfix;
    const int k = blockIdx.x * 256 + threadIdx.x;
    if (k >= M) return;
    const int n = 1 + cnt[k];
    if (n_out) n_out[k] = n;
    const double w = 1.0 / (double)n;
    W[k] = w;
    if (Wfix) Wfix[k] = (unsigned long long)rint(ldexp(w, fix_shift));
}

void gdca_launch_weights(hipStream_t s, const int32_t *cnt, int M, int fix_shift, int32_t *n_out, double *W,
                         unsigned long long *Wfix)
{
    (gdca_launch<k_weights_args, k_weights<1>, k_weights<GDCA_MAXB>>(dim3((M + 255) / 256), dim3(256), 0, s, k_weights_mk(cnt, M, fix_shift, n_out, W, Wfix)));
}

struct k_fix_weights_args {
    const double *W;
    int M;
    int fix_shift;
    unsigned long long *Wfix;
    gdca_dev_scalars *sc;
};
static inline k_fix_weights_args k_fix_weights_mk(const double *W, int M, int fix_shift, unsigned long long *Wfix, gdca_dev_scalars *sc)
{
    return k_fix_weights_args{W, M, fix_shift, Wfix, sc};
}
template <int CAP>
__global__ __launch_bounds__(256) void k_fix_weights(const BatchArgs<k_fix_weights_args, CAP> B_)
{
    GDCA_MEMBER(B_);
    const double *__restrict__ W = a_.W;
    int M = a_.M;
    int fix_shift = a_.fix_shift;
    unsigned long long *__restrict__ Wfix = a_.Wfix;
    gdca_dev_scalars *sc = a_.sc;
    const int k = blockIdx.x * 256 + threadIdx.x;
    if (k >= M) return;
    const double w = W[k];
    const bool ok = w >= 0.0 && w <= 1.0;
    if (!ok) atomicOr(&sc->bad_symbol, GDCA_BAD_WEIGHT);
    Wfix[k] = ok ? (unsigned long long)rint(ldexp(w, fix_shift)) : 0ull;
}

void gdca_launch_fix_weights(hipStream_t s, const double *W, int M, int fix_shift, unsigned long long *Wfix,
                             gdca_dev_scalars *sc)
{
    (gdca_launch<k_fix_weights_args, k_fix_weights<1>, k_fix_weights<GDCA_MAXB>>(dim3((M + 255) / 256), dim3(256), 0, s, k_fix_weights_mk(W, M, fix_shift, Wfix, sc)));
}

#define MEFF_FRAC 84
struct k_meff_args {
    const double *W;
    int M;
    gdca_dev_scalars *sc;
};
static inline k_meff_args k_meff_mk(const double *W, int M, gdca_dev_scalars *sc)
{
    return k_meff_args{W, M, sc};
}
template <int CAP>
__global__ __launch_bounds__(1024) void k_meff(const BatchArgs<k_meff_args, CAP> B_)
{
    GDCA_MEMBER(B_);
    const double *__restrict__ W = a_.W;
    int M = a_.M;
    gdca_dev_scalars *sc = a_.sc;
    __shared__ unsigned long long limb[3];
    const int tid = threadIdx.x;
    if (tid < 3) limb[tid] = 0ull;
    __syncthreads();
    unsigned long long l0 = 0ull, l1 = 0ull, l2 = 0ull;
    for (int k0 = tid; k0 < M; k0 += 8 * (int)blockDim.x) {
        double w[8];
#pragma unroll
        for (int u = 0; u < 8; ++u) {
            const int k = k0 + u * (int)blockDim.x;
            w[u] = k < M ? W[k] : 0.0;
        }
#pragma unroll
        for (int u = 0; u < 8; ++u) {
        const unsigned long long b = (unsigned long long)__double_as_longlong(w[u]);
        const int E = (int)((b >> 52) & 0x7ffull);
        unsigned long long m = b & 0xfffffffffffffull;
        int sh = E - 1075 + MEFF_FRAC;
        if (E != 0) m |= 1ull << 52; else sh += 1;
        if (sh < 0) {
            m = sh > -64 ? m >> (-sh) : 0ull;
            sh = 0;
        }
        if (sh > 43) sh = 43;
        const unsigned long long lo = m << sh, hi = sh ? m >> (64 - sh) : 0ull;
        l0 += lo & 0xffffffffull;
        l1 += lo >> 32;
        l2 += hi;
        }
    }
#pragma unroll
    for (int o = 32; o >= 1; o >>= 1) {
        l0 += __shfl_xor(l0, o);
        l1 += __shfl_xor(l1, o);
        l2 += __shfl_xor(l2, o);
    }
    if ((tid & 63) == 0) {
        atomicAdd(&limb[0], l0);
        atomicAdd(&limb[1], l1);
        atomicAdd(&limb[2], l2);
    }
    __syncthreads();
    if (tid == 0) {
        unsigned long long lo = limb[0], hi = limb[2];
        const unsigned long long mid = limb[1];
        const unsigned long long add = mid << 32;
        lo += add;
        hi += (mid >> 32) + (lo < add ? 1ull : 0ull);
        double r;
        if (hi == 0ull && lo < (1ull << 53)) {
            r = ldexp((double)lo, -MEFF_FRAC);
        } else {
            const int p = hi ? 127 - __builtin_clzll(hi) : 63 - __builtin_clzll(lo);
            const int shift = p - 52;
            unsigned long long kept, rem_hi, rem_lo, half_hi, half_lo;
            if (shift >= 64) {
                kept = hi >> (shift - 64);
                rem_hi = shift > 64 ? hi & ((1ull << (shift - 64)) - 1ull) : 0ull;
                rem_lo = lo;
            } else {
                kept = (lo >> shift) | (hi << (64 - shift));
                rem_hi = 0ull;
                rem_lo = lo & ((1ull << shift) - 1ull);
            }
            if (shift - 1 >= 64) {
                half_hi = 1ull << (shift - 1 - 64);
                half_lo = 0ull;
            } else {
                half_hi = 0ull;
                half_lo = 1ull << (shift - 1);
            }
            const bool above = rem_hi > half_hi || (rem_hi == half_hi && rem_lo > half_lo);
            const bool tie = rem_hi == half_hi && rem_lo == half_lo;
            if (above || (tie && (kept & 1ull))) ++kept;
            r = ldexp((double)kept, shift - MEFF_FRAC);
        }
        sc->Meff = r;
    }
}

void gdca_launch_meff(hipStream_t s, const double *W, int M, gdca_dev_scalars *sc)
{
    (gdca_launch<k_meff_args, k_meff<1>, k_meff<GDCA_MAXB>>(dim3(1), dim3(1024), 0, s, k_meff_mk(W, M, sc)));
}
```

### gaussdca.jl_amd/csrc/k_theta.hip

```cpp
#include "gdca_internal.h"
#include "gdca_launch.h"

struct k_relayout_args {
    const int8_t *Z;
    int8_t *Zt;
    int8_t *Zc;
    int N;
    int M;
    int TJ;
};
static inline k_relayout_args k_relayout_mk(const int8_t *Z, int8_t *Zt, int8_t *Zc, int N, int M, int TJ)
{
    return k_relayout_args{Z, Zt, Zc, N, M, TJ};
}
template <int CAP>
__global__ __launch_bounds__(256) void k_relayout(const BatchArgs<k_relayout_args, CAP> B_)
{
    GDCA_MEMBER(B_);
    const int8_t *__restrict__ Z = a_.Z;
    int8_t *__restrict__ Zt = a_.Zt;
    int8_t *__restrict__ Zc = a_.Zc;
    int N = a_.N;
    int M = a_.M;
    int TJ = a_.TJ;
    __shared__ uint32_t tile[64][17];
    const int k0 = blockIdx.y * 64, c0 = blockIdx.x * 64;
    const int t = threadIdx.x;
    if (((N & 3) == 0) && ((reinterpret_cast<uintptr_t>(Z) & 3) == 0)) {
        const int d = t & 15, c = c0 + 4 * d;
#pragma unroll
        for (int r = 0; r < 4; ++r) {
            const int kl = r * 16 + (t >> 4), k = k0 + kl;
            uint32_t v = 0;
            if (k < M && c < N) v = *reinterpret_cast<const uint32_t *>(Z + (size_t)k * N + c);
            tile[kl][d] = v;
        }
    } else {
        uint8_t *tb = reinterpret_cast<uint8_t *>(&tile[0][0]);
        const int tx = t & 63, ty = t >> 6;
#pragma unroll
        for (int r = 0; r < 16; ++r) {
            const int kl = r * 4 + ty, k = k0 + kl, c = c0 + tx;
            tb[kl * 68 + tx] = (k < M && c < N) ? (uint8_t)Z[(size_t)k * N + c] : (uint8_t)0;
        }
    }
    __syncthreads();
    {
        const int q16 = TJ >> 4;
        const int blk = t / (64 * q16), rem = t % (64 * q16);
        const int kl = rem / q16, h = rem % q16;
        const int k = k0 + kl, cb = c0 / TJ + blk;
        if (k < M && cb * TJ < N) {
            const int d0 = blk * (TJ >> 2) + 4 * h;
            const uint4 v = make_uint4(tile[kl][d0], tile[kl][d0 + 1], tile[kl][d0 + 2], tile[kl][d0 + 3]);
            *reinterpret_cast<uint4 *>(Zc + ((size_t)cb * M + k) * TJ + 16 * h) = v;
        }
    }
    {
        const bool wide = ((M & 3) == 0) && ((reinterpret_cast<uintptr_t>(Zt) & 3) == 0);
        const int bk = t & 15, bc = t >> 4;
        uint32_t r[4];
#pragma unroll
        for (int j = 0; j < 4; ++j) r[j] = tile[4 * bk + j][bc];
        const int k = k0 + 4 * bk;
#pragma unroll
        for (int j = 0; j < 4; ++j) {
            const int i = c0 + 4 * bc + j;
            const uint32_t o = ((r[0] >> (8 * j)) & 255u) | (((r[1] >> (8 * j)) & 255u) << 8) | (((r[2] >> (8 * j)) & 255u) << 16) |
                               (((r[3] >> (8 * j)) & 255u) << 24);
            if (i < N && k < M) {
                int8_t *dst = Zt + (size_t)i * M + k;
                if (wide) {
                    *reinterpret_cast<uint32_t *>(dst) = o;
                } else {
#pragma unroll
                    for (int e = 0; e < 4; ++e)
                        if (k + e < M) dst[e] = (int8_t)((o >> (8 * e)) & 255u);
                }
            }
        }
    }
}

void gdca_launch_relayout(hipStream_t s, const int8_t *Z, int8_t *Zt, int8_t *Zc, int N, int M, int TJ)
{
    dim3 grid((N + 63) / 64, (M + 63) / 64);
    (gdca_launch<k_relayout_args, k_relayout<1>, k_relayout<GDCA_MAXB>>(grid, dim3(256), 0, s, k_relayout_mk(Z, Zt, Zc, N, M, TJ)));
}

#define HIST_THREADS 1024
#define HIST_ROWS 8
struct k_column_hist_args {
    const int8_t *Z;
    uint32_t *out;
    int N;
    int M;
    int seq_per_block;
};
static inline k_column_hist_args k_column_hist_mk(const int8_t *Z, uint32_t *out, int N, int M, int seq_per_block)
{
    return k_column_hist_args{Z, out, N, M, seq_per_block};
}
template <int CAP>
__global__ __launch_bounds__(HIST_THREADS) void k_column_hist(const BatchArgs<k_column_hist_args, CAP> B_)
{
    GDCA_MEMBER(B_);
    const int8_t *__restrict__ Z = a_.Z;
    uint32_t *__restrict__ out = a_.out;
    int N = a_.N;
    int M = a_.M;
    int seq_per_block = a_.seq_per_block;
    constexpr int NW = HIST_THREADS / 64;
    static_assert(HIST_THREADS >= 512, "the store of the counts takes 512 threads");
    __shared__ __attribute__((aligned(16))) uint32_t h[32 * 256];
    const int t = threadIdx.x, lane = t & 63, wv = t >> 6;
    for (int e = t; e < 32 * 256; e += HIST_THREADS) h[e] = 0;
    const int c = blockIdx.x * 256 + 4 * lane;
    const int nv = N - c < 4 ? N - c : 4;
    const int kbeg = blockIdx.y * seq_per_block;
    const int kend = min(M, kbeg + seq_per_block);
    const bool wide = ((N & 3) == 0) && ((reinterpret_cast<uintptr_t>(Z) & 3) == 0);
    __syncthreads();
    if (nv > 0) {
        for (int k = kbeg + wv; k < kend; k += NW * HIST_ROWS) {
            uint32_t v[HIST_ROWS];
#pragma unroll
            for (int u = 0; u < HIST_ROWS; ++u) {
                const int ku = k + u * NW;
                v[u] = 0;
                if (ku < kend) {
                    const int8_t *p = Z + (size_t)ku * N + c;
                    if (wide) {
                        v[u] = *reinterpret_cast<const uint32_t *>(p);
                    } else {
#pragma unroll
                        for (int j = 0; j < 4; ++j)
                            if (j < nv) v[u] |= (uint32_t)(uint8_t)p[j] << (8 * j);
                    }
                }
            }
#pragma unroll
            for (int u = 0; u < HIST_ROWS; ++u) {
                if (k + u * NW < kend) {
#pragma unroll
                    for (int j = 0; j < 4; ++j)
                        if (j < nv) atomicAdd(&h[((v[u] >> (8 * j)) & 31u) * 256 + j * 64 + lane], 1u);
                }
            }
        }
    }
    __syncthreads();
    {
        const int x = t & 255, half = t >> 8;
        const int l = x & 63, j = x >> 6;
        const int col = blockIdx.x * 256 + 4 * l + j;
        if (t < 512 && col < N) {
            uint32_t *dst = out + ((size_t)blockIdx.y * N + col) * 32 + 16 * half;
#pragma unroll
            for (int g = 0; g < 4; ++g) {
                const int z = 16 * half + 4 * g;
                const uint4 o = make_uint4(h[z * 256 + j * 64 + l], h[(z + 1) * 256 + j * 64 + l], h[(z + 2) * 256 + j * 64 + l],
                                           h[(z + 3) * 256 + j * 64 + l]);
                reinterpret_cast<uint4 *>(dst)[g] = o;
            }
        }
    }
}

struct k_column_hist_sum_args {
    const uint32_t *part;
    uint32_t *cnt;
    int total;
    int chunks;
};
static inline k_column_hist_sum_args k_column_hist_sum_mk(const uint32_t *part, uint32_t *cnt, int total, int chunks)
{
    return k_column_hist_sum_args{part, cnt, total, chunks};
}
template <int CAP>
__global__ __launch_bounds__(256) void k_column_hist_sum(const BatchArgs<k_column_hist_sum_args, CAP> B_)
{
    GDCA_MEMBER(B_);
    const uint32_t *__restrict__ part = a_.part;
    uint32_t *__restrict__ cnt = a_.cnt;
    int total = a_.total;
    int chunks = a_.chunks;
    const int e = blockIdx.x * 256 + threadIdx.x;
    if (e >= total) return;
    uint32_t acc = 0;
    int c = 0;
    for (; c + 8 <= chunks; c += 8) {
        uint32_t v[8];
#pragma unroll
        for (int u = 0; u < 8; ++u) v[u] = part[(size_t)(c + u) * total + e];
#pragma unroll
        for (int u = 0; u < 8; ++u) acc += v[u];
    }
    for (; c < chunks; ++c) acc += part[(size_t)c * total + e];
    cnt[e] = acc;
}

static int column_hist_split(int N, int M, int *spb_out)
{
    const int strips = (N + 255) / 256;
    int chunks = (256 + strips - 1) / strips;
    int spb = (M + chunks - 1) / chunks;
    if (spb < 64) spb = 64;
    chunks = (M + spb - 1) / spb;
    if (spb_out) *spb_out = spb;
    return chunks;
}

size_t gdca_column_hist_bytes(int N, int M)
{
    const int chunks = column_hist_split(N, M, nullptr);
    return (size_t)N * 32 * sizeof(uint32_t) * (size_t)(chunks > 1 ? 1 + chunks : 1);
}

void gdca_launch_column_hist(hipStream_t s, const int8_t *Z, uint32_t *cnt, int N, int M)
{
    int spb;
    const int chunks = column_hist_split(N, M, &spb);
    uint32_t *out = chunks > 1 ? cnt + (size_t)N * 32 : cnt;
    (gdca_launch<k_column_hist_args, k_column_hist<1>, k_column_hist<GDCA_MAXB>>(dim3((N + 255) / 256, chunks), dim3(HIST_THREADS), 0, s, k_column_hist_mk(Z, out, N, M, spb)));
    if (chunks > 1)
        (gdca_launch<k_column_hist_sum_args, k_column_hist_sum<1>, k_column_hist_sum<GDCA_MAXB>>(dim3((N * 32 + 255) / 256, 1), dim3(256), 0, s, k_column_hist_sum_mk(out, cnt, N * 32, chunks)));
}

struct k_theta_finalize_args {
    const uint32_t *cnt;
    int N;
    int M;
    double theta_in;
    gdca_dev_scalars *sc;
};
static inline k_theta_finalize_args k_theta_finalize_mk(const uint32_t *cnt, int N, int M, double theta_in, gdca_dev_scalars *sc)
{
    return k_theta_finalize_args{cnt, N, M, theta_in, sc};
}
template <int CAP>
__global__ __launch_bounds__(256) void k_theta_finalize(const BatchArgs<k_theta_finalize_args, CAP> B_)
{
    GDCA_MEMBER(B_);
    const uint32_t *__restrict__ cnt = a_.cnt;
    int N = a_.N;
    int M = a_.M;
    double theta_in = a_.theta_in;
    gdca_dev_scalars *sc = a_.sc;
    __shared__ unsigned long long red[256];
    double theta = theta_in;
    if (theta_in < 0.0) {
        unsigned long long acc = 0;
        for (int e = threadIdx.x; e < N * 32; e += 256) {
            const unsigned long long c = cnt[e];
            acc += c * (c - 1) / 2;
        }
        red[threadIdx.x] = acc;
        __syncthreads();
        for (int w = 128; w > 0; w >>= 1) {
            if (threadIdx.x < w) red[threadIdx.x] += red[threadIdx.x + w];
            __syncthreads();
        }
        if (threadIdx.x == 0) {
            const unsigned long long tot = red[0];
            sc->pair_sum = tot;
            if (M < 2) {
                theta = 0.0;
            } else {
                const double phi = (double)tot / ((double)N * (0.5 * (double)M * (double)(M - 1)));
                const double c = 0.38 * 0.32;
                const double t = c / phi;
                theta = t < 0.5 ? t : 0.5;
            }
        }
    } else if (threadIdx.x == 0) {
        sc->pair_sum = 0;
    }
    if (threadIdx.x == 0) {
        sc->theta = theta;
        sc->thresh = (int)floor(theta * (double)N);
    }
}

void gdca_launch_theta_finalize(hipStream_t s, const uint32_t *cnt, int N, int M, double theta_in,
                                gdca_dev_scalars *sc)
{
    (gdca_launch<k_theta_finalize_args, k_theta_finalize<1>, k_theta_finalize<GDCA_MAXB>>(dim3(1), dim3(256), 0, s, k_theta_finalize_mk(cnt, N, M, theta_in, sc)));
}

struct k_set_thresh_args {
    gdca_dev_scalars *sc;
    int thresh;
};
static inline k_set_thresh_args k_set_thresh_mk(gdca_dev_scalars *sc, int thresh)
{
    return k_set_thresh_args{sc, thresh};
}
template <int CAP>
__global__ void k_set_thresh(const BatchArgs<k_set_thresh_args, CAP> B_)
{
    GDCA_MEMBER(B_);
    gdca_dev_scalars *sc = a_.sc;
    int thresh = a_.thresh;
    sc->thresh = thresh;
}

void gdca_launch_set_thresh(hipStream_t s, gdca_dev_scalars *sc, int thresh)
{
    (gdca_launch<k_set_thresh_args, k_set_thresh<1>, k_set_thresh<GDCA_MAXB>>(dim3(1), dim3(1), 0, s, k_set_thresh_mk(sc, thresh)));
}
```

Measured before the change: 52.18.

## Fuse small weight-stage kernels and make hamming kernel grid-stride persistent

Folds the theta finalize into the column histogram sum kernel using a last-block-arrives pattern, folds the hcnt zero-fill into the bitplane pack kernel, and folds the Meff reduction into the weights kernel. The hamming tile kernels become persistent, launched with a grid capped at 32 blocks per CU and looping over tiles with early exits turned into jumps to the next tile. The aim is to cut kernel-launch and tail overhead in the weights stage. The cost is extra atomics and counters in device scalars, plus a more complex control flow in the hamming kernel.

```diff
diff --git a/gaussdca.jl_amd/csrc/gdca_api.hip b/gaussdca.jl_amd/csrc/gdca_api.hip
--- a/gaussdca.jl_amd/csrc/gdca_api.hip
+++ b/gaussdca.jl_amd/csrc/gdca_api.hip
@@ -856,8 +856,8 @@
     if (fixed_thresh >= 0) {
         gdca_launch_set_thresh(s, sc, fixed_thresh);
     } else {
-        if (theta_in < 0.0) gdca_launch_column_hist(s, Zd, (uint32_t *)ctx->hist.p, N, M);
-        gdca_launch_theta_finalize(s, (const uint32_t *)ctx->hist.p, N, M, theta_in, sc);
+        const bool done = theta_in < 0.0 && gdca_launch_column_hist(s, Zd, (uint32_t *)ctx->hist.p, N, M, sc);
+        if (!done) gdca_launch_theta_finalize(s, (const uint32_t *)ctx->hist.p, N, M, theta_in, sc);
     }
     CHK(check_launch(ctx, "theta"));
     CHK(mark(ctx, T_THETA));
@@ -872,8 +872,7 @@
     CHK(ensure(ctx, ctx->nk, (size_t)M * sizeof(int32_t)));
     CHK(ensure(ctx, ctx->W, (size_t)M * sizeof(double)));
     CHK(ensure(ctx, ctx->Wfix, (size_t)M * sizeof(unsigned long long)));
-    gdca_fill_async(s, ctx->hcnt.p, 0, (size_t)Mt * GDCA_HTILE * sizeof(int32_t));
-    gdca_launch_bitplane_pack(s, Zd, (uint32_t *)ctx->Zb.p, N, M, q, sc);
+    gdca_launch_bitplane_pack(s, Zd, (uint32_t *)ctx->Zb.p, N, M, q, sc, (int32_t *)ctx->hcnt.p);
     if (ctx->tune.force_fallback) {
         gdca_launch_hamming_fallback(s, Zd, (int32_t *)ctx->hcnt.p, N, M, sc);
     } else {
@@ -881,11 +880,10 @@
             if (!(fixed_thresh < 0 && theta_in < 0.0)) gdca_launch_column_hist(s, Zd, (uint32_t *)ctx->hist.p, N, M);
             gdca_launch_hamming_fp4_image(s, Zd, (const uint32_t *)ctx->hist.p, ctx->himg.p, N, M);
         }
-        gdca_launch_hamming(s, (const uint32_t *)ctx->Zb.p, Zd, (int32_t *)ctx->hcnt.p, N, M, sc, ctx->tune.hamming_mode, ctx->hcand.p, fp4 ? ctx->himg.p : nullptr, ctx->tune.ham_cut);
+        gdca_launch_hamming(s, (const uint32_t *)ctx->Zb.p, Zd, (int32_t *)ctx->hcnt.p, N, M, sc, ctx->tune.hamming_mode, ctx->hcand.p, fp4 ? ctx->himg.p : nullptr, ctx->tune.ham_cut, ctx->ncu);
     }
     gdca_launch_weights(s, (const int32_t *)ctx->hcnt.p, M, gdca_fix_shift(M), (int32_t *)ctx->nk.p,
-                        (double *)ctx->W.p, (unsigned long long *)ctx->Wfix.p);
-    gdca_launch_meff(s, (const double *)ctx->W.p, M, sc);
+                        (double *)ctx->W.p, (unsigned long long *)ctx->Wfix.p, sc);
     return check_launch(ctx, "weights");
 }
 
diff --git a/gaussdca.jl_amd/csrc/gdca_internal.h b/gaussdca.jl_amd/csrc/gdca_internal.h
--- a/gaussdca.jl_amd/csrc/gdca_internal.h
+++ b/gaussdca.jl_amd/csrc/gdca_internal.h
@@ -43,6 +43,8 @@
     int ham_cut;
     unsigned ham_alive[64];
     double logdet;
+    unsigned long long theta_sum, meff_limb[3];
+    unsigned theta_arrived, meff_arrived;
 };
 
 struct gdca_tuning {
@@ -86,25 +88,24 @@
 
 void gdca_launch_relayout(hipStream_t s, const int8_t *Z, int8_t *Zt, int8_t *Zc, int N, int M, int TJ);
 size_t gdca_column_hist_bytes(int N, int M);
-void gdca_launch_column_hist(hipStream_t s, const int8_t *Z, uint32_t *cnt, int N, int M);
+bool gdca_launch_column_hist(hipStream_t s, const int8_t *Z, uint32_t *cnt, int N, int M, gdca_dev_scalars *sc = nullptr);
 void gdca_launch_theta_finalize(hipStream_t s, const uint32_t *cnt, int N, int M, double theta_in,
                                 gdca_dev_scalars *sc);
 void gdca_launch_set_thresh(hipStream_t s, gdca_dev_scalars *sc, int thresh);
 
 size_t gdca_bitplane_bytes(int N, int M);
 void gdca_launch_bitplane_pack(hipStream_t s, const int8_t *Z, uint32_t *Zb, int N, int M, int q,
-                               gdca_dev_scalars *sc);
+                               gdca_dev_scalars *sc, int32_t *cnt0);
 size_t gdca_hamming_cand_cap(int M);
 size_t gdca_fp4_image_bytes(int N, int M);
 void gdca_launch_hamming_fp4_image(hipStream_t s, const int8_t *Z, const uint32_t *hist, void *img, int N, int M);
 void gdca_launch_hamming_fp4_probe(hipStream_t s, const void *img, int N, int M, int nprobe, gdca_dev_scalars *sc);
 void gdca_launch_hamming_fp4(hipStream_t s, const void *img, int N, int M, gdca_dev_scalars *sc, void *cand_list, unsigned cap);
 void gdca_launch_hamming(hipStream_t s, const uint32_t *Zb, const int8_t *Z, int32_t *cnt, int N, int M, gdca_dev_scalars *sc, int force,
-                         void *cand_list, void *fp4_img, int cut);
+                         void *cand_list, void *fp4_img, int cut, int ncu);
 void gdca_launch_hamming_fallback(hipStream_t s, const int8_t *Z, int32_t *cnt, int N, int M, const gdca_dev_scalars *sc);
 void gdca_launch_weights(hipStream_t s, const int32_t *cnt, int M, int fix_shift, int32_t *n_out, double *W,
-                         unsigned long long *Wfix);
-void gdca_launch_meff(hipStream_t s, const double *W, int M, gdca_dev_scalars *sc);
+                         unsigned long long *Wfix, gdca_dev_scalars *sc);
 void gdca_launch_fix_weights(hipStream_t s, const double *W, int M, int fix_shift, unsigned long long *Wfix,
                              gdca_dev_scalars *sc);
 int gdca_fix_shift(int M);
diff --git a/gaussdca.jl_amd/csrc/k_hamming.hip b/gaussdca.jl_amd/csrc/k_hamming.hip
--- a/gaussdca.jl_amd/csrc/k_hamming.hip
+++ b/gaussdca.jl_amd/csrc/k_hamming.hip
@@ -23,10 +23,11 @@
     int NW;
     int q;
     gdca_dev_scalars *sc;
+    int32_t *cnt0;
 };
-static inline k_bitplane_pack_args k_bitplane_pack_mk(const int8_t *Z, uint32_t *Zb, int N, int M, int NW, int q, gdca_dev_scalars *sc)
-{
-    return k_bitplane_pack_args{Z, Zb, N, M, NW, q, sc};
+static inline k_bitplane_pack_args k_bitplane_pack_mk(const int8_t *Z, uint32_t *Zb, int N, int M, int NW, int q, gdca_dev_scalars *sc, int32_t *cnt0)
+{
+    return k_bitplane_pack_args{Z, Zb, N, M, NW, q, sc, cnt0};
 }
 template <int CAP>
 __global__ __launch_bounds__(128) void k_bitplane_pack(const BatchArgs<k_bitplane_pack_args, CAP> B_)
@@ -43,6 +44,7 @@
     const uint32_t over = (0x7fu - (uint32_t)q) * 0x01010101u;
     const int tile = blockIdx.x, w = blockIdx.y, kl = threadIdx.x;
     const int k = tile * GDCA_HTILE + kl;
+    if (w == 0 && a_.cnt0) a_.cnt0[k] = 0;
     uint32_t pl[NPLANES];
 #pragma unroll
     for (int p = 0; p < NPLANES; ++p) pl[p] = 0;
@@ -82,10 +84,10 @@
     if (bad) atomicOr(&sc->bad_symbol, GDCA_BAD_ALIGNMENT);
 }
 
-void gdca_launch_bitplane_pack(hipStream_t s, const int8_t *Z, uint32_t *Zb, int N, int M, int q, gdca_dev_scalars *sc)
+void gdca_launch_bitplane_pack(hipStream_t s, const int8_t *Z, uint32_t *Zb, int N, int M, int q, gdca_dev_scalars *sc, int32_t *cnt0)
 {
     const int Mt = (M + GDCA_HTILE - 1) / GDCA_HTILE, NW = (N + 31) / 32;
-    (gdca_launch<k_bitplane_pack_args, k_bitplane_pack<1>, k_bitplane_pack<GDCA_MAXB>>(dim3(Mt, NW), dim3(128), 0, s, k_bitplane_pack_mk(Z, Zb, N, M, NW, q, sc)));
+    (gdca_launch<k_bitplane_pack_args, k_bitplane_pack<1>, k_bitplane_pack<GDCA_MAXB>>(dim3(Mt, NW), dim3(128), 0, s, k_bitplane_pack_mk(Z, Zb, N, M, NW, q, sc, cnt0)));
 }
 
 __device__ __forceinline__ void tri_decode(int t, int Mt, int &I, int &J)
@@ -103,6 +105,7 @@
 
 #define HAM_BOUND_PLANES 3
 #define HAM_CAND_CAP 1024
+#define HAM_GRID_PER_CU 32
 
 __shared__ int hm_any[3];
 __shared__ unsigned hm_tile_n, hm_tile_base;
@@ -215,6 +218,14 @@
 {
     return k_hamming_args{Zb, cnt, NW, M, Mt, sc, cand_list, cand_cap};
 }
+#define HAM_TID()                                                                                              \
+    ({                                                                                                         \
+        int t_;                                                                                                \
+        asm volatile("v_mbcnt_lo_u32_b32 %0, -1, 0\n\tv_mbcnt_hi_u32_b32 %0, -1, %0" : "=v"(t_));              \
+        t_ += wave0 * 64;                                                                                      \
+        asm volatile("" : "+v"(t_));                                                                           \
+        t_;                                                                                                    \
+    })
 template <int CAP, int NP, bool PROBE>
 __global__ __launch_bounds__(256, (NP < NPLANES && !PROBE) ? 4 : 3) void k_hamming(const BatchArgs<k_hamming_args, CAP> B_)
 {
@@ -238,18 +249,27 @@
     __shared__ __attribute__((aligned(16))) uint32_t Bs[NP][WCHUNK][GDCA_HTILE];
     __shared__ int rc[GDCA_HTILE], cc[GDCA_HTILE];
 
+    const long long ntile = (long long)Mt * (Mt + 1) / 2;
+    const int wave0 = __builtin_amdgcn_readfirstlane((int)threadIdx.x >> 6);
+    constexpr bool CUTTING = NP < NPLANES && !PROBE;
+    int cut0 = NW;
+    if constexpr (CUTTING) {
+        const int c = sc->ham_cut;
+        if (c > 0 && c < NW && NW < HAM_CUT_MAX_NW) cut0 = c;
+    }
+    for (long long t = PROBE ? ((long long)blockIdx.x * ntile) / gridDim.x : (long long)blockIdx.x;;) {
+    {
+    const int tid = HAM_TID(), tx = tid & 15, ty = tid >> 4;
     int I, J;
-    tri_decode(PROBE ? (int)(((long long)blockIdx.x * ((long long)Mt * (Mt + 1) / 2)) / gridDim.x) : (int)blockIdx.x, Mt, I, J);
-    const int tid = threadIdx.x, tx = tid & 15, ty = tid >> 4;
+    int Mt_ = Mt;
+    asm volatile("" : "+s"(Mt_));
+    tri_decode((int)t, Mt_, I, J);
     if (tid < GDCA_HTILE) {
         rc[tid] = 0;
         cc[tid] = 0;
     }
-    if (tid == 0) {
-        hm_any[0] = 0;
-        hm_any[1] = 0;
-        hm_tile_n = 0u;
-    }
+    if (tid < 2) hm_any[tid] = 0;
+    if (tid == 2) hm_tile_n = 0u;
     int any_calls = 0;
 
     uint32_t acc[8][8];
@@ -274,12 +294,7 @@
     const uint32_t *Ag = Zb + (size_t)I * NPLANES * NW * GDCA_HTILE;
     const uint32_t *Bg = Zb + (size_t)J * NPLANES * NW * GDCA_HTILE;
 
-    constexpr bool CUTTING = NP < NPLANES && !PROBE;
-    int cut = NW;
-    if constexpr (CUTTING) {
-        const int c = sc->ham_cut;
-        if (c > 0 && c < NW && NW < HAM_CUT_MAX_NW) cut = c;
-    }
+    int cut = cut0;
     bool sparse = false;
     if constexpr (PROBE)
         if (tid < HAM_ALIVE_SLOTS) hm_alive[tid] = 0u;
@@ -345,6 +360,7 @@
         }
         if constexpr (CUTTING) {
             if (w0 + w == cut && cut < NW) {
+                const int tid = HAM_TID(), tx = tid & 15, ty = tid >> 4;
                 const uint32_t rc0 = ((uint32_t)(ty * 8) << 25) | ((uint32_t)(tx * 4) << 18);
                 uint32_t *const mylist = hm_list[tid >> 6];
                 int wcount = 0;
@@ -391,6 +407,8 @@
         }
     }
 
+    {
+    const int tid = HAM_TID(), tx = tid & 15, ty = tid >> 4;
     const bool diag = (I == J);
     if constexpr (PROBE) {
         int cand = 0;
@@ -408,7 +426,7 @@
         if (tid < HAM_ALIVE_SLOTS && hm_alive[tid]) atomicAdd(&sc->ham_alive[tid], hm_alive[tid]);
         return;
     }
-    if (all_beyond) return;
+    if (all_beyond) goto next_tile;
     if constexpr (CUTTING) {
         if (sparse) {
             const int lane = tid & 63, nmine = hm_wave_n[tid >> 6];
@@ -437,11 +455,11 @@
                         left |= (int)d < thresh;
                     }
                 }
-                if (w0 + WCHUNK < NW && !wg_any(left, any_calls)) return;
+                if (w0 + WCHUNK < NW && !wg_any(left, any_calls)) goto next_tile;
             }
             unsigned mine = 0u;
             for (int e = lane; e < nmine; e += 64) mine += (int)(mylist[e] & HAM_ENT_DIST) < thresh;
-            if (!wg_any(mine != 0u, any_calls)) return;
+            if (!wg_any(mine != 0u, any_calls)) goto next_tile;
             const unsigned off = mine ? atomicAdd(&hm_tile_n, mine) : 0u;
             __syncthreads();
             if (tid == 0) {
@@ -457,7 +475,7 @@
                     ++slot;
                 }
             }
-            return;
+            goto next_tile;
         }
     }
     if constexpr (NP < NPLANES) {
@@ -466,7 +484,7 @@
         for (int r = 0; r < 8; ++r)
 #pragma unroll
             for (int c = 0; c < 8; ++c) mn = min(mn, acc[r][c]);
-        unsigned long long cand = 0ull;
+        uint32_t cand_lo = 0u, cand_hi = 0u;
         if ((int)mn < thresh) {
 #pragma unroll
             for (int r = 0; r < 8; ++r)
@@ -474,10 +492,13 @@
                 for (int c = 0; c < 8; ++c) {
                     const int lc = (c < 4) ? (tx * 4 + c) : (64 + tx * 4 + (c - 4));
                     const int gr = I * GDCA_HTILE + ty * 8 + r, gc = J * GDCA_HTILE + lc;
-                    if ((int)acc[r][c] < thresh && gr < M && gc < M && (diag ? gr < gc : true)) cand |= 1ull << (8 * r + c);
-                }
-        }
-        if (!wg_any(cand != 0ull, any_calls)) return;
+                    if ((int)acc[r][c] < thresh && gr < M && gc < M && (diag ? gr < gc : true)) {
+                        if (r < 4) cand_lo |= 1u << (8 * r + c); else cand_hi |= 1u << (8 * (r - 4) + c);
+                    }
+                }
+        }
+        unsigned long long cand = (unsigned long long)cand_hi << 32 | cand_lo;
+        if (!wg_any(cand != 0ull, any_calls)) goto next_tile;
         const unsigned mine = (unsigned)__builtin_popcountll(cand);
         const unsigned off = mine ? atomicAdd(&hm_tile_n, mine) : 0u;
         __syncthreads();
@@ -494,7 +515,7 @@
             ++slot;
             cand &= cand - 1;
         }
-        return;
+        goto next_tile;
     }
 
     if constexpr (NP == NPLANES) {
@@ -533,6 +554,14 @@
     } else if (!diag) {
         const int v = cc[tid - GDCA_HTILE];
         if (v) atomicAdd(&cnt[J * GDCA_HTILE + tid - GDCA_HTILE], v);
+    }
+    }
+    }
+    next_tile:
+        if constexpr (PROBE) return;
+        t += gridDim.x;
+        if (t >= ntile) return;
+        __syncthreads();
     }
 }
 
@@ -566,10 +595,11 @@
 }
 
 void gdca_launch_hamming(hipStream_t s, const uint32_t *Zb, const int8_t *Z, int32_t *cnt, int N, int M, gdca_dev_scalars *sc, int force,
-                         void *cand_list, void *fp4_img, int cut)
+                         void *cand_list, void *fp4_img, int cut, int ncu)
 {
     const int Mt = (M + GDCA_HTILE - 1) / GDCA_HTILE, NW = (N + 31) / 32;
     const long long ntile = (long long)Mt * (Mt + 1) / 2;
+    const unsigned tgrid = (unsigned)std::min<long long>(ntile, (long long)HAM_GRID_PER_CU * (ncu > 0 ? ncu : 256));
     int2 *list = (int2 *)cand_list;
     const unsigned cap = (unsigned)gdca_hamming_cand_cap(M);
     const int nprobe = (int)std::min<long long>(ntile, 192);
@@ -586,10 +616,10 @@
     const int form = decided ? (force < 0 ? 0 : force) : -1;
     if (fp4_img && (form == 2 || form < 0)) gdca_launch_hamming_fp4(s, fp4_img, N, M, sc, list, cap);
     if (form == 1 || form < 0)
-        (gdca_launch<k_hamming_args, k_hamming<1, HAM_BOUND_PLANES, false>, k_hamming<GDCA_MAXB, HAM_BOUND_PLANES, false>>(dim3((unsigned)ntile), dim3(256), 0, s, k_hamming_mk(Zb, cnt, NW, M, Mt, sc, list, cap)));
+        (gdca_launch<k_hamming_args, k_hamming<1, HAM_BOUND_PLANES, false>, k_hamming<GDCA_MAXB, HAM_BOUND_PLANES, false>>(dim3(tgrid), dim3(256), 0, s, k_hamming_mk(Zb, cnt, NW, M, Mt, sc, list, cap)));
     if (form != 0)
         (gdca_launch<k_hamming_refine_args, k_hamming_refine<1>, k_hamming_refine<GDCA_MAXB>>(dim3(2048), dim3(256), 0, s, k_hamming_refine_mk(Z, (const int2 *)list, cap, N, cnt, (const gdca_dev_scalars *)sc)));
-    (gdca_launch<k_hamming_args, k_hamming<1, NPLANES, false>, k_hamming<GDCA_MAXB, NPLANES, false>>(dim3((unsigned)ntile), dim3(256), 0, s, k_hamming_mk(Zb, cnt, NW, M, Mt, sc, list, cap)));
+    (gdca_launch<k_hamming_args, k_hamming<1, NPLANES, false>, k_hamming<GDCA_MAXB, NPLANES, false>>(dim3(tgrid), dim3(256), 0, s, k_hamming_mk(Zb, cnt, NW, M, Mt, sc, list, cap)));
 }
 
 struct k_hamming_bytes_args {
@@ -647,6 +677,58 @@
     return sh < 58 ? sh : 58;
 }
 
+#define MEFF_FRAC 84
+__device__ __forceinline__ void meff_add(double w, unsigned long long &l0, unsigned long long &l1, unsigned long long &l2)
+{
+    const unsigned long long b = (unsigned long long)__double_as_longlong(w);
+    const int E = (int)((b >> 52) & 0x7ffull);
+    unsigned long long m = b & 0xfffffffffffffull;
+    int sh = E - 1075 + MEFF_FRAC;
+    if (E != 0) m |= 1ull << 52; else sh += 1;
+    if (sh < 0) {
+        m = sh > -64 ? m >> (-sh) : 0ull;
+        sh = 0;
+    }
+    if (sh > 43) sh = 43;
+    const unsigned long long lo = m << sh, hi = sh ? m >> (64 - sh) : 0ull;
+    l0 += lo & 0xffffffffull;
+    l1 += lo >> 32;
+    l2 += hi;
+}
+__device__ double meff_round(unsigned long long limb0, unsigned long long limb1, unsigned long long limb2)
+{
+    unsigned long long lo = limb0, hi = limb2;
+    const unsigned long long mid = limb1;
+    const unsigned long long add = mid << 32;
+    lo += add;
+    hi += (mid >> 32) + (lo < add ? 1ull : 0ull);
+    if (hi == 0ull && lo < (1ull << 53)) return ldexp((double)lo, -MEFF_FRAC);
+    const int p = hi ? 127 - __builtin_clzll(hi) : 63 - __builtin_clzll(lo);
+    const int shift = p - 52;
+    unsigned long long kept, rem_hi, rem_lo, half_hi, half_lo;
+    if (shift >= 64) {
+        kept = hi >> (shift - 64);
+        rem_hi = shift > 64 ? hi & ((1ull << (shift - 64)) - 1ull) : 0ull;
+        rem_lo = lo;
+    } else {
+        kept = (lo >> shift) | (hi << (64 - shift));
+        rem_hi = 0ull;
+        rem_lo = lo & ((1ull << shift) - 1ull);
+    }
+    if (shift - 1 >= 64) {
+        half_hi = 1ull << (shift - 1 - 64);
+        half_lo = 0ull;
+    } else {
+        half_hi = 0ull;
+        half_lo = 1ull << (shift - 1);
+    }
+    const bool above = rem_hi > half_hi || (rem_hi == half_hi && rem_lo > half_lo);
+    const bool tie = rem_hi == half_hi && rem_lo == half_lo;
+    if (above || (tie && (kept & 1ull))) ++kept;
+    return ldexp((double)kept, shift - MEFF_FRAC);
+}
+
+#define WEIGHTS_THREADS 1024
 struct k_weights_args {
     const int32_t *cnt;
     int M;
@@ -654,13 +736,14 @@
     int32_t *n_out;
     double *W;
     unsigned long long *Wfix;
+    gdca_dev_scalars *sc;
 };
-static inline k_weights_args k_weights_mk(const int32_t *cnt, int M, int fix_shift, int32_t *n_out, double *W, unsigned long long *Wfix)
-{
-    return k_weights_args{cnt, M, fix_shift, n_out, W, Wfix};
+static inline k_weights_args k_weights_mk(const int32_t *cnt, int M, int fix_shift, int32_t *n_out, double *W, unsigned long long *Wfix, gdca_dev_scalars *sc)
+{
+    return k_weights_args{cnt, M, fix_shift, n_out, W, Wfix, sc};
 }
 template <int CAP>
-__global__ __launch_bounds__(256) void k_weights(const BatchArgs<k_weights_args, CAP> B_)
+__global__ __launch_bounds__(WEIGHTS_THREADS) void k_weights(const BatchArgs<k_weights_args, CAP> B_)
 {
     GDCA_MEMBER(B_);
     const int32_t *__restrict__ cnt = a_.cnt;
@@ -669,19 +752,52 @@
     int32_t *__restrict__ n_out = a_.n_out;
     double *__restrict__ W = a_.W;
     unsigned long long *__restrict__ Wfix = a_.Wfix;
-    const int k = blockIdx.x * 256 + threadIdx.x;
-    if (k >= M) return;
-    const int n = 1 + cnt[k];
-    if (n_out) n_out[k] = n;
-    const double w = 1.0 / (double)n;
-    W[k] = w;
-    if (Wfix) Wfix[k] = (unsigned long long)rint(ldexp(w, fix_shift));
+    gdca_dev_scalars *sc = a_.sc;
+    __shared__ unsigned long long limb[3];
+    const int tid = threadIdx.x, k = blockIdx.x * WEIGHTS_THREADS + tid;
+    unsigned long long l0 = 0ull, l1 = 0ull, l2 = 0ull;
+    if (k < M) {
+        const int n = 1 + cnt[k];
+        if (n_out) n_out[k] = n;
+        const double w = 1.0 / (double)n;
+        W[k] = w;
+        if (Wfix) Wfix[k] = (unsigned long long)rint(ldexp(w, fix_shift));
+        meff_add(w, l0, l1, l2);
+    }
+    if (!sc) return;
+    if (tid < 3) limb[tid] = 0ull;
+    __syncthreads();
+#pragma unroll
+    for (int o = 32; o >= 1; o >>= 1) {
+        l0 += __shfl_xor(l0, o);
+        l1 += __shfl_xor(l1, o);
+        l2 += __shfl_xor(l2, o);
+    }
+    if ((tid & 63) == 0) {
+        atomicAdd(&limb[0], l0);
+        atomicAdd(&limb[1], l1);
+        atomicAdd(&limb[2], l2);
+    }
+    __syncthreads();
+    if (tid == 0) {
+        atomicAdd(&sc->meff_limb[0], limb[0]);
+        atomicAdd(&sc->meff_limb[1], limb[1]);
+        atomicAdd(&sc->meff_limb[2], limb[2]);
+        __threadfence();
+        if (atomicAdd(&sc->meff_arrived, 1u) == gridDim.x - 1u) {
+            __threadfence();
+            const unsigned long long s0 = atomicExch(&sc->meff_limb[0], 0ull), s1 = atomicExch(&sc->meff_limb[1], 0ull),
+                                     s2 = atomicExch(&sc->meff_limb[2], 0ull);
+            atomicExch(&sc->meff_arrived, 0u);
+            sc->Meff = meff_round(s0, s1, s2);
+        }
+    }
 }
 
 void gdca_launch_weights(hipStream_t s, const int32_t *cnt, int M, int fix_shift, int32_t *n_out, double *W,
-                         unsigned long long *Wfix)
-{
-    (gdca_launch<k_weights_args, k_weights<1>, k_weights<GDCA_MAXB>>(dim3((M + 255) / 256), dim3(256), 0, s, k_weights_mk(cnt, M, fix_shift, n_out, W, Wfix)));
+                         unsigned long long *Wfix, gdca_dev_scalars *sc)
+{
+    (gdca_launch<k_weights_args, k_weights<1>, k_weights<GDCA_MAXB>>(dim3((M + WEIGHTS_THREADS - 1) / WEIGHTS_THREADS), dim3(WEIGHTS_THREADS), 0, s, k_weights_mk(cnt, M, fix_shift, n_out, W, Wfix, sc)));
 }
 
 struct k_fix_weights_args {
@@ -717,105 +833,3 @@
 {
     (gdca_launch<k_fix_weights_args, k_fix_weights<1>, k_fix_weights<GDCA_MAXB>>(dim3((M + 255) / 256), dim3(256), 0, s, k_fix_weights_mk(W, M, fix_shift, Wfix, sc)));
 }
-
-#define MEFF_FRAC 84
-struct k_meff_args {
-    const double *W;
-    int M;
-    gdca_dev_scalars *sc;
-};
-static inline k_meff_args k_meff_mk(const double *W, int M, gdca_dev_scalars *sc)
-{
-    return k_meff_args{W, M, sc};
-}
-template <int CAP>
-__global__ __launch_bounds__(1024) void k_meff(const BatchArgs<k_meff_args, CAP> B_)
-{
-    GDCA_MEMBER(B_);
-    const double *__restrict__ W = a_.W;
-    int M = a_.M;
-    gdca_dev_scalars *sc = a_.sc;
-    __shared__ unsigned long long limb[3];
-    const int tid = threadIdx.x;
-    if (tid < 3) limb[tid] = 0ull;
-    __syncthreads();
-    unsigned long long l0 = 0ull, l1 = 0ull, l2 = 0ull;
-    for (int k0 = tid; k0 < M; k0 += 8 * (int)blockDim.x) {
-        double w[8];
-#pragma unroll
-        for (int u = 0; u < 8; ++u) {
-            const int k = k0 + u * (int)blockDim.x;
-            w[u] = k < M ? W[k] : 0.0;
-        }
-#pragma unroll
-        for (int u = 0; u < 8; ++u) {
-        const unsigned long long b = (unsigned long long)__double_as_longlong(w[u]);
-        const int E = (int)((b >> 52) & 0x7ffull);
-        unsigned long long m = b & 0xfffffffffffffull;
-        int sh = E - 1075 + MEFF_FRAC;
-        if (E != 0) m |= 1ull << 52; else sh += 1;
-        if (sh < 0) {
-            m = sh > -64 ? m >> (-sh) : 0ull;
-            sh = 0;
-        }
-        if (sh > 43) sh = 43;
-        const unsigned long long lo = m << sh, hi = sh ? m >> (64 - sh) : 0ull;
-        l0 += lo & 0xffffffffull;
-        l1 += lo >> 32;
-        l2 += hi;
-        }
-    }
-#pragma unroll
-    for (int o = 32; o >= 1; o >>= 1) {
-        l0 += __shfl_xor(l0, o);
-        l1 += __shfl_xor(l1, o);
-        l2 += __shfl_xor(l2, o);
-    }
-    if ((tid & 63) == 0) {
-        atomicAdd(&limb[0], l0);
-        atomicAdd(&limb[1], l1);
-        atomicAdd(&limb[2], l2);
-    }
-    __syncthreads();
-    if (tid == 0) {
-        unsigned long long lo = limb[0], hi = limb[2];
-        const unsigned long long mid = limb[1];
-        const unsigned long long add = mid << 32;
-        lo += add;
-        hi += (mid >> 32) + (lo < add ? 1ull : 0ull);
-        double r;
-        if (hi == 0ull && lo < (1ull << 53)) {
-            r = ldexp((double)lo, -MEFF_FRAC);
-        } else {
-            const int p = hi ? 127 - __builtin_clzll(hi) : 63 - __builtin_clzll(lo);
-            const int shift = p - 52;
-            unsigned long long kept, rem_hi, rem_lo, half_hi, half_lo;
-            if (shift >= 64) {
-                kept = hi >> (shift - 64);
-                rem_hi = shift > 64 ? hi & ((1ull << (shift - 64)) - 1ull) : 0ull;
-                rem_lo = lo;
-            } else {
-                kept = (lo >> shift) | (hi << (64 - shift));
-                rem_hi = 0ull;
-                rem_lo = lo & ((1ull << shift) - 1ull);
-            }
-            if (shift - 1 >= 64) {
-                half_hi = 1ull << (shift - 1 - 64);
-                half_lo = 0ull;
-            } else {
-                half_hi = 0ull;
-                half_lo = 1ull << (shift - 1);
-            }
-            const bool above = rem_hi > half_hi || (rem_hi == half_hi && rem_lo > half_lo);
-            const bool tie = rem_hi == half_hi && rem_lo == half_lo;
-            if (above || (tie && (kept & 1ull))) ++kept;
-            r = ldexp((double)kept, shift - MEFF_FRAC);
-        }
-        sc->Meff = r;
-    }
-}
-
-void gdca_launch_meff(hipStream_t s, const double *W, int M, gdca_dev_scalars *sc)
-{
-    (gdca_launch<k_meff_args, k_meff<1>, k_meff<GDCA_MAXB>>(dim3(1), dim3(1024), 0, s, k_meff_mk(W, M, sc)));
-}
diff --git a/gaussdca.jl_amd/csrc/k_theta.hip b/gaussdca.jl_amd/csrc/k_theta.hip
--- a/gaussdca.jl_amd/csrc/k_theta.hip
+++ b/gaussdca.jl_amd/csrc/k_theta.hip
@@ -167,15 +167,26 @@
     }
 }
 
+__device__ __forceinline__ double theta_auto(unsigned long long tot, int N, int M)
+{
+    if (M < 2) return 0.0;
+    const double phi = (double)tot / ((double)N * (0.5 * (double)M * (double)(M - 1)));
+    const double c = 0.38 * 0.32;
+    const double t = c / phi;
+    return t < 0.5 ? t : 0.5;
+}
+
 struct k_column_hist_sum_args {
     const uint32_t *part;
     uint32_t *cnt;
     int total;
     int chunks;
-};
-static inline k_column_hist_sum_args k_column_hist_sum_mk(const uint32_t *part, uint32_t *cnt, int total, int chunks)
-{
-    return k_column_hist_sum_args{part, cnt, total, chunks};
+    int N, M;
+    gdca_dev_scalars *sc;
+};
+static inline k_column_hist_sum_args k_column_hist_sum_mk(const uint32_t *part, uint32_t *cnt, int total, int chunks, int N, int M, gdca_dev_scalars *sc)
+{
+    return k_column_hist_sum_args{part, cnt, total, chunks, N, M, sc};
 }
 template <int CAP>
 __global__ __launch_bounds__(256) void k_column_hist_sum(const BatchArgs<k_column_hist_sum_args, CAP> B_)
@@ -185,19 +196,44 @@
     uint32_t *__restrict__ cnt = a_.cnt;
     int total = a_.total;
     int chunks = a_.chunks;
+    gdca_dev_scalars *sc = a_.sc;
+    __shared__ unsigned long long wg_sum;
     const int e = blockIdx.x * 256 + threadIdx.x;
-    if (e >= total) return;
     uint32_t acc = 0;
-    int c = 0;
-    for (; c + 8 <= chunks; c += 8) {
-        uint32_t v[8];
-#pragma unroll
-        for (int u = 0; u < 8; ++u) v[u] = part[(size_t)(c + u) * total + e];
-#pragma unroll
-        for (int u = 0; u < 8; ++u) acc += v[u];
-    }
-    for (; c < chunks; ++c) acc += part[(size_t)c * total + e];
-    cnt[e] = acc;
+    if (e < total) {
+        int c = 0;
+        for (; c + 8 <= chunks; c += 8) {
+            uint32_t v[8];
+#pragma unroll
+            for (int u = 0; u < 8; ++u) v[u] = part[(size_t)(c + u) * total + e];
+#pragma unroll
+            for (int u = 0; u < 8; ++u) acc += v[u];
+        }
+        for (; c < chunks; ++c) acc += part[(size_t)c * total + e];
+        cnt[e] = acc;
+    }
+    if (!sc) return;
+    if (threadIdx.x == 0) wg_sum = 0ull;
+    __syncthreads();
+    const unsigned long long c = acc;
+    unsigned long long pairs = c * (c - 1) / 2;
+#pragma unroll
+    for (int o = 32; o >= 1; o >>= 1) pairs += __shfl_xor(pairs, o);
+    if ((threadIdx.x & 63) == 0) atomicAdd(&wg_sum, pairs);
+    __syncthreads();
+    if (threadIdx.x == 0) {
+        atomicAdd(&sc->theta_sum, wg_sum);
+        __threadfence();
+        if (atomicAdd(&sc->theta_arrived, 1u) == gridDim.x - 1u) {
+            __threadfence();
+            const unsigned long long tot = atomicExch(&sc->theta_sum, 0ull);
+            atomicExch(&sc->theta_arrived, 0u);
+            const double theta = theta_auto(tot, a_.N, a_.M);
+            sc->pair_sum = tot;
+            sc->theta = theta;
+            sc->thresh = (int)floor(theta * (double)a_.N);
+        }
+    }
 }
 
 static int column_hist_split(int N, int M, int *spb_out)
@@ -217,14 +253,15 @@
     return (size_t)N * 32 * sizeof(uint32_t) * (size_t)(chunks > 1 ? 1 + chunks : 1);
 }
 
-void gdca_launch_column_hist(hipStream_t s, const int8_t *Z, uint32_t *cnt, int N, int M)
+bool gdca_launch_column_hist(hipStream_t s, const int8_t *Z, uint32_t *cnt, int N, int M, gdca_dev_scalars *sc)
 {
     int spb;
     const int chunks = column_hist_split(N, M, &spb);
     uint32_t *out = chunks > 1 ? cnt + (size_t)N * 32 : cnt;
     (gdca_launch<k_column_hist_args, k_column_hist<1>, k_column_hist<GDCA_MAXB>>(dim3((N + 255) / 256, chunks), dim3(HIST_THREADS), 0, s, k_column_hist_mk(Z, out, N, M, spb)));
     if (chunks > 1)
-        (gdca_launch<k_column_hist_sum_args, k_column_hist_sum<1>, k_column_hist_sum<GDCA_MAXB>>(dim3((N * 32 + 255) / 256, 1), dim3(256), 0, s, k_column_hist_sum_mk(out, cnt, N * 32, chunks)));
+        (gdca_launch<k_column_hist_sum_args, k_column_hist_sum<1>, k_column_hist_sum<GDCA_MAXB>>(dim3((N * 32 + 255) / 256, 1), dim3(256), 0, s, k_column_hist_sum_mk(out, cnt, N * 32, chunks, N, M, sc)));
+    return chunks > 1 && sc != nullptr;
 }
 
 struct k_theta_finalize_args {
@@ -264,14 +301,7 @@
         if (threadIdx.x == 0) {
             const unsigned long long tot = red[0];
             sc->pair_sum = tot;
-            if (M < 2) {
-                theta = 0.0;
-            } else {
-                const double phi = (double)tot / ((double)N * (0.5 * (double)M * (double)(M - 1)));
-                const double c = 0.38 * 0.32;
-                const double t = c / phi;
-                theta = t < 0.5 ? t : 0.5;
-            }
+            theta = theta_auto(tot, N, M);
         }
     } else if (threadIdx.x == 0) {
         sc->pair_sum = 0;
```

New measurement: 52.40 (median of 6 runs). About the same (+0.4%).
